# fgvieira/ngsLD

Measured on AMD Instinct MI355X. Metric: SNP-pair EM-LD computations/sec @ n_ind=500, higher is better.
Workload: dtype f64

## Files before the change

include/ngsld.h:

```cpp
#ifndef NGSLD_H
#define NGSLD_H

#include <stddef.h>
#include <stdint.h>

#ifdef __cplusplus
extern "C" {
#endif

typedef struct ngsld_ctx ngsld_ctx;

enum {
  NGSLD_OK = 0,
  NGSLD_ERR_INVALID = -1,
  NGSLD_ERR_DEVICE = -2,
  NGSLD_ERR_NOMEM = -3,
  NGSLD_ERR_NAN = -4,
  NGSLD_ERR_MAF_RANGE = -5,
  NGSLD_ERR_SINK = -6,
  NGSLD_ERR_UNSUPPORTED = -7
};

typedef struct {
  uint64_t max_kb_dist;
// ... 19 lines not shown
  uint32_t n_iter;
} ngsld_rec_ext;

typedef struct {
  uint32_t s1, s2_begin, count, reserved;
  uint64_t mask;
  uint64_t first_record;
} ngsld_item;

typedef struct {
  uint64_t s1_begin, s1_end;
  uint64_t n_pairs;
  uint64_t n_items;
  const ngsld_item *items;
  const ngsld_rec_std *std;
  const ngsld_rec_ext *ext;
  const char *text;
  uint64_t text_len;
} ngsld_batch;

typedef int (*ngsld_sink_fn)(void *user, const ngsld_batch *batch);

typedef int (*ngsld_read_sites_fn)(void *user, uint64_t site_begin, uint64_t n_sites, double *dst);

const char *ngsld_version(void);

int ngsld_create(int device, ngsld_ctx **ctx);
void ngsld_destroy(ngsld_ctx *ctx);
const char *ngsld_last_error(const ngsld_ctx *ctx);

int ngsld_set_geno_raw(ngsld_ctx *ctx, const double *gl_raw, uint64_t n_sites, uint64_t n_ind, int log_scale,
                       int ignore_miss_data, int on_device);
typedef struct {
  int32_t log_scale;
  int32_t ignore_miss_data;
  int32_t on_device;
  int32_t text_semantics;
  int32_t call_geno;
  int32_t per_individual_only;
  double N_thresh;
  double call_thresh;
} ngsld_geno_opts;
int ngsld_set_geno_raw_opts(ngsld_ctx *ctx, const double *gl_raw, uint64_t n_sites, uint64_t n_ind,
                            const ngsld_geno_opts *opts);
int ngsld_set_geno_lkl(ngsld_ctx *ctx, const double *geno_lkl, const double *maf, uint64_t n_sites, uint64_t n_ind,
                       int on_device);
int ngsld_get_maf(ngsld_ctx *ctx, double *maf_out);
int ngsld_set_pos_dist(ngsld_ctx *ctx, const double *pos_dist);

int ngsld_plan(ngsld_ctx *ctx, const ngsld_params *params, uint64_t *n_pairs);
int ngsld_plan_rows(ngsld_ctx *ctx, const uint64_t **row_off, const uint32_t **row_end);

int ngsld_run(ngsld_ctx *ctx, uint64_t s1_begin, uint64_t s1_end, ngsld_sink_fn sink, void *user);

int ngsld_set_text_output(ngsld_ctx *ctx, const char *const *labels, int enable);

int ngsld_reserve_text_buffers(ngsld_ctx *ctx, uint64_t bytes_per_row);

int ngsld_set_replay_source(ngsld_ctx *ctx, ngsld_read_sites_fn read, void *user);
int ngsld_set_replay_matrix(ngsld_ctx *ctx, const double *values);
int ngsld_set_replay(ngsld_ctx *ctx, int enable);
int ngsld_replay_stats(ngsld_ctx *ctx, uint64_t *pairs, uint64_t *sites);

int ngsld_set_exact_store(ngsld_ctx *ctx, int mode);
typedef struct {
  uint64_t pairs_flagged;
  uint64_t pairs_replayed;
  uint64_t pairs_on_device;
  uint64_t pairs_on_host;
  uint64_t sites_reevaluated;
  int32_t exact_store;
  int32_t text_rows_patched;
  double exact_store_build_s;
  uint64_t sites_degenerate;
} ngsld_replay_stats_t;
int ngsld_replay_info(ngsld_ctx *ctx, ngsld_replay_stats_t *out);

int ngsld_run_device(ngsld_ctx *ctx, uint64_t s1_begin, uint64_t s1_end, void *d_std, void *d_ext, void *hip_stream);
int ngsld_finish_device(ngsld_ctx *ctx);

int ngsld_last_kernel_time(ngsld_ctx *ctx, double *total_ms, uint64_t *n_launches, uint64_t *n_pairs);

const char *ngsld_pair_kernel(const ngsld_ctx *ctx);
int ngsld_describe_dispatch(uint64_t n_ind, int ignore_miss_data, char *buf, size_t buf_len);

int ngsld_set_tuning(ngsld_ctx *ctx, uint32_t pairs_per_item, uint64_t batch_pairs);

int ngsld_selftest(ngsld_ctx *ctx);

int ngsld_selftest_format(ngsld_ctx *ctx, uint64_t n, const ngsld_rec_std *std, const ngsld_rec_ext *ext, const double *dist,
                          const double *maf1, const double *maf2, char *text, uint64_t text_cap, uint64_t *row_len,
                          int32_t *needs_host);
int ngsld_selftest_printed(ngsld_ctx *ctx, uint64_t n, const double *x, int32_t precision, int32_t weight_type,
                           double min_weight, int64_t *micro, int32_t *micro_ok, int64_t *label, int32_t *label_rc);

typedef struct {
  uint64_t row_begin, row_end;
  uint64_t site_end;
} ngsld_slab;

int ngsld_window_ends(const double *pos_dist, uint64_t n_sites, const ngsld_params *params, uint32_t *row_end);

int ngsld_plan_slabs(const double *pos_dist, uint64_t n_sites, const ngsld_params *params, uint64_t max_slab_sites,
                     ngsld_slab *slabs, uint64_t cap, uint64_t *n_slabs);

uint64_t ngsld_slab_sites_for_budget(uint64_t n_ind, uint64_t budget_bytes);
uint64_t ngsld_sites_for_budget(uint64_t n_ind, uint64_t budget_bytes, int matrix_copies);

int ngsld_streamed_replay_info(ngsld_replay_stats_t *out);

int ngsld_set_memory_budget(int device, uint64_t bytes);

int ngsld_device_memory(int device, uint64_t *free_bytes, uint64_t *total_bytes);


int ngsld_run_streamed(int device, uint64_t n_sites, uint64_t n_ind, const double *pos_dist,
                       const ngsld_params *params, const ngsld_geno_opts *opts, uint64_t max_slab_sites,
                       ngsld_read_sites_fn read, void *read_user, double *maf_out, ngsld_sink_fn sink,
                       void *sink_user, uint64_t *n_pairs, uint64_t *n_slabs, char *err, size_t errlen);

int ngsld_run_streamed_text(int device, uint64_t n_sites, uint64_t n_ind, const double *pos_dist,
                            const ngsld_params *params, const ngsld_geno_opts *opts, uint64_t max_slab_sites,
                            ngsld_read_sites_fn read, void *read_user, double *maf_out, ngsld_sink_fn sink,
                            void *sink_user, uint64_t *n_pairs, uint64_t *n_slabs, char *err, size_t errlen,
                            const char *const *labels, int text_output);


int ngsld_plan_parts(const double *pos_dist, uint64_t n_sites, const ngsld_params *params, int n_parts, ngsld_slab *parts);

typedef int (*ngsld_multi_sink_fn)(void *user, int part, const ngsld_batch *batch);

int ngsld_run_multi(const int *devices, int n_devices, uint64_t n_sites, uint64_t n_ind, const double *pos_dist,
                    const ngsld_params *params, const ngsld_geno_opts *opts, const double *gl_raw,
                    ngsld_read_sites_fn read, void *read_user, double *maf_out, ngsld_multi_sink_fn sink, void *sink_user,
                    const char *const *labels, int text_output, uint64_t *pairs_per_part, char *err, size_t errlen);

enum { NGSLD_DIST_NONE = 0, NGSLD_DIST_UPLOAD = 1, NGSLD_DIST_PEER_COPY = 2, NGSLD_DIST_RCCL = 3 };
int ngsld_multi_last_distribution(void);

int ngsld_rccl_selftest(int device, uint64_t bytes, char *err, size_t errlen);

typedef struct {
  uint32_t struct_size;
  int32_t field;
  double max_kb_dist;
  double min_weight;
  int32_t weight_type;
  int32_t keep_heavy;
  int32_t precision;
  int32_t reserved;
  const char *const *subset;
  uint64_t n_subset;
} ngsld_prune_params;

typedef struct {
  uint32_t struct_size;
  uint32_t reserved;
  uint64_t pairs;
  uint64_t nodes, edges;
  uint64_t kept, excluded;
  uint64_t rounds;
  uint64_t host_nodes, host_edges, host_steps;
  double pairs_ms, edges_ms, graph_ms, rounds_ms, host_ms, total_ms;
} ngsld_prune_stats;

int ngsld_prune(ngsld_ctx *ctx, const ngsld_prune_params *params, const char *const *labels, uint8_t *site_state,
// ... 105 lines not shown
```

ngsld_amd/capi.py:

```python
from __future__ import annotations

import ctypes as C
import os
import subprocess

import numpy as np

PKG_DIR = os.path.dirname(os.path.abspath(__file__))
REPO_DIR = os.path.dirname(PKG_DIR)
LIB_PATH = os.environ.get("NGSLD_LIB") or os.path.join(PKG_DIR, "libngsld.so")
CLI_PATH = os.path.join(PKG_DIR, "bin", "ngsLD")

OK, ERR_INVALID, ERR_DEVICE, ERR_NOMEM, ERR_NAN, ERR_MAF_RANGE, ERR_SINK, ERR_UNSUPPORTED = 0, -1, -2, -3, -4, -5, -6, -7


class Params(C.Structure):
    _fields_ = [("max_kb_dist", C.c_uint64), ("max_snp_dist", C.c_uint64), ("min_maf", C.c_double),
                ("ignore_miss_data", C.c_int32), ("extend_out", C.c_int32), ("rnd_sample", C.c_double),
                ("seed", C.c_uint64), ("first_row", C.c_uint64)]


class GenoOpts(C.Structure):
    _fields_ = [("log_scale", C.c_int32), ("ignore_miss_data", C.c_int32), ("on_device", C.c_int32),
                ("text_semantics", C.c_int32), ("call_geno", C.c_int32), ("per_individual_only", C.c_int32),
                ("N_thresh", C.c_double), ("call_thresh", C.c_double)]


REC_STD = np.dtype([("r2_ExpG", "<f8"), ("D", "<f8"), ("Dp", "<f8"), ("r2", "<f8")])
REC_EXT = np.dtype([("hap", "<f8", (4,)), ("n_ind_data", "<u4"), ("n_iter", "<u4")])


ITEM = np.dtype([("s1", "<u4"), ("s2_begin", "<u4"), ("count", "<u4"), ("reserved", "<u4"), ("mask", "<u8"),
                 ("first_record", "<u8")])


class Batch(C.Structure):
    _fields_ = [("s1_begin", C.c_uint64), ("s1_end", C.c_uint64), ("n_pairs", C.c_uint64), ("n_items", C.c_uint64),
                ("items", C.c_void_p), ("std", C.c_void_p), ("ext", C.c_void_p), ("text", C.c_void_p),
                ("text_len", C.c_uint64)]


def items_to_pairs(items: np.ndarray) -> tuple[np.ndarray, np.ndarray]:
    if len(items) == 0:
        return np.zeros(0, dtype=np.uint64), np.zeros(0, dtype=np.uint64)
    bits = (items["mask"][:, None] >> np.arange(64, dtype=np.uint64)[None, :]) & np.uint64(1)
    bits &= (np.arange(64)[None, :] < items["count"][:, None]).astype(np.uint64)
    idx, c = np.nonzero(bits)
    return items["s1"][idx].astype(np.uint64), (items["s2_begin"][idx].astype(np.uint64) + c.astype(np.uint64))


def items_from_pairs(s1: np.ndarray, s2: np.ndarray, span: int = 64) -> np.ndarray:
    s1, s2 = np.asarray(s1, dtype=np.int64), np.asarray(s2, dtype=np.int64)
    chunk = (s2 - s1 - 1) // span
    key = s1 * (1 << 32) + chunk
    uniq, first, inv = np.unique(key, return_index=True, return_inverse=True)
    items = np.zeros(len(uniq), dtype=ITEM)
    items["s1"] = s1[first]
    items["s2_begin"] = s1[first] + 1 + chunk[first] * span
    items["first_record"] = first
    np.bitwise_or.at(items["mask"], inv, np.uint64(1) << (s2 - items["s2_begin"][inv]).astype(np.uint64))
    last = np.zeros(len(uniq), dtype=np.int64)
    np.maximum.at(last, inv, s2 - items["s2_begin"][inv].astype(np.int64))
    items["count"] = last + 1
    return items


SINK_FN = C.CFUNCTYPE(C.c_int, C.c_void_p, C.POINTER(Batch))
MULTI_SINK_FN = C.CFUNCTYPE(C.c_int, C.c_void_p, C.c_int, C.POINTER(Batch))
READ_FN = C.CFUNCTYPE(C.c_int, C.c_void_p, C.c_uint64, C.c_uint64, C.c_void_p)
SLAB = np.dtype([("row_begin", "<u8"), ("row_end", "<u8"), ("site_end", "<u8")])

SYMBOLS = [
    "ngsld_version", "ngsld_create", "ngsld_destroy", "ngsld_last_error", "ngsld_set_geno_raw",
    "ngsld_set_geno_raw_opts", "ngsld_set_geno_lkl",
    "ngsld_get_maf", "ngsld_set_pos_dist", "ngsld_plan", "ngsld_plan_rows", "ngsld_run", "ngsld_run_device", "ngsld_set_text_output",
    "ngsld_set_replay_source", "ngsld_set_replay_matrix", "ngsld_set_replay", "ngsld_replay_stats", "ngsld_finish_device",
    "ngsld_set_exact_store", "ngsld_replay_info",
    "ngsld_plan_parts", "ngsld_run_multi", "ngsld_multi_last_distribution", "ngsld_rccl_selftest",
    "ngsld_last_kernel_time", "ngsld_pair_kernel", "ngsld_describe_dispatch", "ngsld_set_tuning", "ngsld_selftest", "ngsld_selftest_format",
    "ngsld_selftest_printed", "ngsld_reserve_text_buffers",
    "ngsld_window_ends", "ngsld_plan_slabs", "ngsld_slab_sites_for_budget", "ngsld_sites_for_budget", "ngsld_streamed_replay_info", "ngsld_set_memory_budget", "ngsld_device_memory", "ngsld_run_streamed", "ngsld_run_streamed_text",
    "ngsld_host_read_geno_bin_range",
    "ngsld_host_set_threads", "ngsld_host_read_pos", "ngsld_host_pos_dist", "ngsld_host_label", "ngsld_host_free_pos", "ngsld_host_pos_slice",
    "ngsld_host_geno_size_ok", "ngsld_host_read_geno_bin", "ngsld_host_read_geno_text", "ngsld_host_format_header", "ngsld_host_format_pair",
    "ngsld_host_format_double", "ngsld_host_write_batch", "ngsld_host_replay_pair", "ngsld_host_missing_call_log",
    "ngsld_host_gz_open", "ngsld_host_gz_close",
    "ngsld_prune", "ngsld_host_prune_graph", "ngsld_host_prune_label",
    "ngsld_decay", "ngsld_decay_bins", "ngsld_host_decay_fit",
    "ngsld_blocks", "ngsld_blocks_sites", "ngsld_blocks_matrix", "ngsld_blocks_text",
    "ngsld_site_ld", "ngsld_site_ld_get",
    "ngsld_clusters", "ngsld_clusters_sites", "ngsld_clusters_table",
]


class ReplayStats(C.Structure):
    _fields_ = [("pairs_flagged", C.c_uint64), ("pairs_replayed", C.c_uint64), ("pairs_on_device", C.c_uint64),
                ("pairs_on_host", C.c_uint64), ("sites_reevaluated", C.c_uint64), ("exact_store", C.c_int32),
                ("text_rows_patched", C.c_int32), ("exact_store_build_s", C.c_double), ("sites_degenerate", C.c_uint64)]


class PruneParams(C.Structure):
    _fields_ = [("struct_size", C.c_uint32), ("field", C.c_int32), ("max_kb_dist", C.c_double), ("min_weight", C.c_double),
                ("weight_type", C.c_int32), ("keep_heavy", C.c_int32), ("precision", C.c_int32), ("reserved", C.c_int32),
                ("subset", C.POINTER(C.c_char_p)), ("n_subset", C.c_uint64)]


class PruneStats(C.Structure):
    _fields_ = [("struct_size", C.c_uint32), ("reserved", C.c_uint32), ("pairs", C.c_uint64), ("nodes", C.c_uint64),
                ("edges", C.c_uint64), ("kept", C.c_uint64), ("excluded", C.c_uint64), ("rounds", C.c_uint64),
                ("host_nodes", C.c_uint64), ("host_edges", C.c_uint64), ("host_steps", C.c_uint64),
                ("pairs_ms", C.c_double), ("edges_ms", C.c_double), ("graph_ms", C.c_double), ("rounds_ms", C.c_double),
                ("host_ms", C.c_double), ("total_ms", C.c_double)]


class DecayParams(C.Structure):
    _fields_ = [("struct_size", C.c_uint32), ("fields", C.c_uint32), ("bin_size", C.c_double), ("max_kb_dist", C.c_double),
                ("min_maf", C.c_double)]


class DecayStats(C.Structure):
    _fields_ = [("struct_size", C.c_uint32), ("lds", C.c_uint32), ("pairs", C.c_uint64), ("pairs_counted", C.c_uint64),
                ("bins", C.c_uint64), ("bin_slots", C.c_uint64), ("chunks", C.c_uint64), ("pairs_ms", C.c_double),
                ("bin_ms", C.c_double), ("total_ms", C.c_double)]


class BlocksParams(C.Structure):
    _fields_ = [("struct_size", C.c_uint32), ("fields", C.c_uint32), ("chr", C.c_char_p), ("start", C.c_uint64),
                ("end", C.c_uint64)]


class BlocksStats(C.Structure):
    _fields_ = [("struct_size", C.c_uint32), ("reserved", C.c_uint32), ("members", C.c_uint64), ("sites", C.c_uint64),
                ("pairs", C.c_uint64), ("pairs_in_region", C.c_uint64), ("cells_na", C.c_uint64), ("host_rows", C.c_uint64),
                ("chunks", C.c_uint64), ("pairs_ms", C.c_double), ("scatter_ms", C.c_double), ("format_ms", C.c_double),
                ("total_ms", C.c_double)]


class SiteLdParams(C.Structure):
    _fields_ = [("struct_size", C.c_uint32), ("fields", C.c_uint32), ("max_kb_dist", C.c_double), ("min_maf", C.c_double),
                ("linked_min", C.c_double), ("abs_value", C.c_int32), ("reserved", C.c_int32)]


class SiteLdStats(C.Structure):
    _fields_ = [("struct_size", C.c_uint32), ("lds", C.c_uint32), ("pairs", C.c_uint64), ("pairs_counted", C.c_uint64),
                ("sites_with_pairs", C.c_uint64), ("chunks", C.c_uint64), ("pairs_ms", C.c_double), ("site_ms", C.c_double),
                ("total_ms", C.c_double)]


class ClustersParams(C.Structure):
    _fields_ = [("struct_size", C.c_uint32), ("field", C.c_int32), ("max_kb_dist", C.c_double), ("min_maf", C.c_double),
                ("min_weight", C.c_double), ("abs_value", C.c_int32), ("reserved", C.c_int32)]


class ClustersStats(C.Structure):
    _fields_ = [("struct_size", C.c_uint32), ("reserved", C.c_uint32), ("pairs", C.c_uint64), ("nodes", C.c_uint64),
                ("edges", C.c_uint64), ("clusters", C.c_uint64), ("clusters_multi", C.c_uint64), ("largest", C.c_uint64),
                ("chunks", C.c_uint64), ("union_launches", C.c_uint64), ("pairs_ms", C.c_double), ("union_ms", C.c_double),
                ("finish_ms", C.c_double), ("total_ms", C.c_double)]


TEXT_FN = C.CFUNCTYPE(C.c_int, C.c_void_p, C.c_void_p, C.c_uint64)


class DecayFitResult(C.Structure):
    _fields_ = [("rate", C.c_double), ("ld_max", C.c_double), ("ld_min", C.c_double), ("sse", C.c_double),
                ("n_bins", C.c_uint64)]


DECAY_FIELDS = ("r2_ExpG", "D", "Dp", "r2")


class NgsldError(RuntimeError):
    def __init__(self, code: int, msg: str):
        super().__init__(f"ngsld error {code}: {msg}")
        self.code = code
        self.msg = msg


def build(force: bool = False, jobs: int = 8) -> None:
    csrc = os.path.join(PKG_DIR, "csrc")
    if force:
        subprocess.check_call(["make", "-s", "-C", csrc, "clean"])
    subprocess.check_call(["make", "-s", f"-j{jobs}", "-C", csrc, "all"])


_lib = None


def lib() -> C.CDLL:
    global _lib
    if _lib is None:
        if not os.path.exists(LIB_PATH):
            raise FileNotFoundError(f"{LIB_PATH} is missing: run ngsld_amd.capi.build() (or make -C ngsld_amd/csrc); "
                                    "there is no fallback implementation")
        L = C.CDLL(LIB_PATH)
        vp, u64, dbl = C.c_void_p, C.c_uint64, C.c_double
        L.ngsld_version.restype = C.c_char_p
        L.ngsld_create.argtypes = [C.c_int, C.POINTER(vp)]
        L.ngsld_destroy.argtypes = [vp]
        L.ngsld_destroy.restype = None
        L.ngsld_last_error.argtypes = [vp]
        L.ngsld_last_error.restype = C.c_char_p
        L.ngsld_set_geno_raw.argtypes = [vp, vp, u64, u64, C.c_int, C.c_int, C.c_int]
        L.ngsld_set_geno_raw_opts.argtypes = [vp, vp, u64, u64, C.POINTER(GenoOpts)]
        L.ngsld_set_geno_lkl.argtypes = [vp, vp, vp, u64, u64, C.c_int]
        L.ngsld_get_maf.argtypes = [vp, vp]
        L.ngsld_set_pos_dist.argtypes = [vp, vp]
        L.ngsld_plan.argtypes = [vp, C.POINTER(Params), C.POINTER(u64)]
        L.ngsld_plan_rows.argtypes = [vp, C.POINTER(C.POINTER(C.c_uint64)), C.POINTER(C.POINTER(C.c_uint32))]
        L.ngsld_run.argtypes = [vp, u64, u64, SINK_FN, vp]
        L.ngsld_run_device.argtypes = [vp, u64, u64, vp, vp, vp]
        if hasattr(L, "ngsld_set_replay_source"):
            L.ngsld_set_replay_source.argtypes = [vp, READ_FN, vp]
            if hasattr(L, "ngsld_set_replay_matrix"):
                L.ngsld_set_replay_matrix.argtypes = [vp, vp]
            L.ngsld_set_replay.argtypes = [vp, C.c_int]
            L.ngsld_replay_stats.argtypes = [vp, C.POINTER(u64), C.POINTER(u64)]
        if hasattr(L, "ngsld_replay_info"):
            L.ngsld_set_exact_store.argtypes = [vp, C.c_int]
            L.ngsld_replay_info.argtypes = [vp, C.POINTER(ReplayStats)]
            L.ngsld_finish_device.argtypes = [vp]
        if hasattr(L, "ngsld_set_text_output"):
            L.ngsld_set_text_output.argtypes = [vp, C.POINTER(C.c_char_p), C.c_int]
        L.ngsld_last_kernel_time.argtypes = [vp, C.POINTER(dbl), C.POINTER(u64), C.POINTER(u64)]
        L.ngsld_set_tuning.argtypes = [vp, C.c_uint32, u64]
        if hasattr(L, "ngsld_pair_kernel"):
            L.ngsld_pair_kernel.argtypes = [vp]
            L.ngsld_pair_kernel.restype = C.c_char_p
        L.ngsld_selftest.argtypes = [vp]
        if hasattr(L, "ngsld_selftest_format"):
            L.ngsld_selftest_format.argtypes = [vp, u64, vp, vp, vp, vp, vp, C.c_char_p, u64, vp, C.POINTER(C.c_int32)]
            L.ngsld_selftest_printed.argtypes = [vp, u64, vp, C.c_int32, C.c_int32, dbl, vp, vp, vp, vp]
        L.ngsld_window_ends.argtypes = [vp, u64, C.POINTER(Params), vp]
        L.ngsld_plan_slabs.argtypes = [vp, u64, C.POINTER(Params), u64, vp, u64, C.POINTER(u64)]
        L.ngsld_slab_sites_for_budget.argtypes = [u64, u64]
        L.ngsld_slab_sites_for_budget.restype = u64
        if hasattr(L, "ngsld_sites_for_budget"):
            L.ngsld_sites_for_budget.argtypes = [u64, u64, C.c_int]
            L.ngsld_sites_for_budget.restype = u64
        L.ngsld_device_memory.argtypes = [C.c_int, C.POINTER(u64), C.POINTER(u64)]
        L.ngsld_run_streamed.argtypes = [C.c_int, u64, u64, vp, C.POINTER(Params), C.POINTER(GenoOpts), u64, READ_FN, vp,
                                         vp, SINK_FN, vp, C.POINTER(u64), C.POINTER(u64), C.c_char_p, C.c_size_t]
        if hasattr(L, "ngsld_run_multi"):
            L.ngsld_plan_parts.argtypes = [vp, u64, C.POINTER(Params), C.c_int, vp]
            L.ngsld_run_multi.argtypes = [C.POINTER(C.c_int), C.c_int, u64, u64, vp, C.POINTER(Params), C.POINTER(GenoOpts),
                                          vp, READ_FN, vp, vp, MULTI_SINK_FN, vp, C.POINTER(C.c_char_p), C.c_int,
                                          C.POINTER(u64), C.c_char_p, C.c_size_t]
        if hasattr(L, "ngsld_multi_last_distribution"):
            L.ngsld_multi_last_distribution.argtypes = []
        if hasattr(L, "ngsld_rccl_selftest"):
            L.ngsld_rccl_selftest.argtypes = [C.c_int, u64, C.c_char_p, C.c_size_t]
        L.ngsld_host_read_geno_bin_range.argtypes = [C.c_char_p, u64, u64, u64, vp, C.c_char_p, C.c_size_t]
        L.ngsld_host_set_threads.argtypes = [C.c_int]
        L.ngsld_host_set_threads.restype = None
        L.ngsld_host_read_pos.argtypes = [C.c_char_p, C.c_int, u64, C.POINTER(vp), C.c_char_p, C.c_size_t]
        L.ngsld_host_pos_dist.argtypes = [vp]
        L.ngsld_host_pos_dist.restype = C.POINTER(dbl)
        L.ngsld_host_label.argtypes = [vp, u64]
        L.ngsld_host_label.restype = C.c_char_p
        L.ngsld_host_free_pos.argtypes = [vp]
        L.ngsld_host_free_pos.restype = None
        L.ngsld_host_pos_slice.argtypes = [vp, u64, u64]
        L.ngsld_host_pos_slice.restype = vp
        L.ngsld_host_geno_size_ok.argtypes = [u64, u64, u64]
        L.ngsld_host_read_geno_bin.argtypes = [C.c_char_p, u64, u64, vp, C.c_char_p, C.c_size_t]
        L.ngsld_host_read_geno_text.argtypes = [C.c_char_p, C.c_int, C.c_int, u64, u64, vp, C.POINTER(C.c_int),
                                                C.c_char_p, C.c_size_t]
        L.ngsld_host_format_header.argtypes = [C.c_char_p, C.c_size_t, C.c_int]
        L.ngsld_host_format_header.restype = C.c_size_t
        L.ngsld_host_format_pair.argtypes = [C.c_char_p, C.c_size_t, C.c_char_p, C.c_char_p, dbl, vp, vp, dbl, dbl]
        L.ngsld_host_format_pair.restype = C.c_size_t
        L.ngsld_host_format_double.argtypes = [C.c_char_p, C.c_size_t, dbl, C.c_int]
        L.ngsld_host_format_double.restype = C.c_size_t
        L.ngsld_host_write_batch.argtypes = [C.POINTER(Batch), vp, vp, vp, C.c_int, C.c_int]
        L.ngsld_host_replay_pair.argtypes = [vp, vp, u64, C.POINTER(GenoOpts), vp, vp, vp]
        if hasattr(L, "ngsld_host_gz_open"):
            L.ngsld_host_gz_open.argtypes = [C.c_char_p, C.c_int, C.POINTER(vp), C.POINTER(C.c_int)]
            L.ngsld_host_gz_close.argtypes = [vp]
        if hasattr(L, "ngsld_prune"):
            L.ngsld_prune.argtypes = [vp, C.POINTER(PruneParams), C.POINTER(C.c_char_p), vp, C.POINTER(PruneStats)]
            L.ngsld_host_prune_graph.argtypes = [u64, vp, u64, vp, vp, vp, C.c_int, vp, C.POINTER(u64)]
            L.ngsld_host_prune_label.argtypes = [dbl, C.c_int, C.c_char, C.POINTER(C.c_int64)]
        if hasattr(L, "ngsld_decay"):
            L.ngsld_decay.argtypes = [vp, C.POINTER(DecayParams), C.POINTER(DecayStats)]
            L.ngsld_decay_bins.argtypes = [vp, u64, vp, vp, vp, C.POINTER(u64)]
            L.ngsld_host_decay_fit.argtypes = [u64, vp, vp, C.c_int, dbl, dbl, C.POINTER(DecayFitResult)]
        if hasattr(L, "ngsld_blocks"):
            L.ngsld_blocks.argtypes = [vp, C.POINTER(BlocksParams), C.POINTER(C.c_char_p), C.POINTER(BlocksStats)]
            L.ngsld_blocks_sites.argtypes = [vp, u64, vp, C.POINTER(u64)]
            L.ngsld_blocks_matrix.argtypes = [vp, C.c_int, vp, vp]
            L.ngsld_blocks_text.argtypes = [vp, C.c_int, TEXT_FN, vp, C.POINTER(BlocksStats)]
        if hasattr(L, "ngsld_site_ld"):
            L.ngsld_site_ld.argtypes = [vp, C.POINTER(SiteLdParams), C.POINTER(SiteLdStats)]
            L.ngsld_site_ld_get.argtypes = [vp, C.c_int, vp, vp, vp, vp, vp]
        if hasattr(L, "ngsld_clusters"):
            L.ngsld_clusters.argtypes = [vp, C.POINTER(ClustersParams), C.POINTER(ClustersStats)]
            L.ngsld_clusters_sites.argtypes = [vp, vp]
            L.ngsld_clusters_table.argtypes = [vp, u64, u64, vp, vp, vp, vp, vp, vp, vp, vp, vp, C.POINTER(u64)]
        _lib = L
    return _lib


def prune_label(x: float, prec: int = 4, weight_type: str = "a") -> int | None:
    out = C.c_int64()
    rc = lib().ngsld_host_prune_label(float(x), prec, weight_type.encode(), C.byref(out))
    if rc == ERR_INVALID:
        return None
    if rc != OK:
        raise NgsldError(rc, "label out of range")
    return out.value


def decay_fit(dist, values, field: str = "r2", n_ind: float = 0, recomb_rate: float = 1.0) -> dict:
    d = np.ascontiguousarray(dist, dtype=np.float64)
    v = np.ascontiguousarray(values, dtype=np.float64)
    if d.shape != v.shape or d.ndim != 1:
        raise ValueError("dist and values must be 1-D arrays of one length")
# ... 541 lines not shown
                    exts.append(np.frombuffer(C.string_at(b.ext, n * REC_EXT.itemsize), dtype=REC_EXT).copy())
            items = np.frombuffer(C.string_at(b.items, b.n_items * ITEM.itemsize), dtype=ITEM) if b.n_items else \
                np.zeros(0, dtype=ITEM)
            a, bb = items_to_pairs(items)
            assert len(a) == n
            if len(items):
                assert np.array_equal(items["first_record"], np.concatenate([[0], np.cumsum(
                    [bin(int(m)).count("1") for m in items["mask"]])[:-1]]).astype(np.uint64))
            s1s.append(a)
            s2s.append(bb)
            return 0

        cb = SINK_FN(sink)
        self._check(self._L.ngsld_run(self._h, s1_begin, s1_end, cb, None))
        cat = lambda xs, dt: np.concatenate(xs) if xs else np.zeros(0, dtype=dt)
        return (cat(s1s, np.uint64), cat(s2s, np.uint64), cat(stds, REC_STD),
                cat(exts, REC_EXT) if self.extend_out else None)

    def run_to_fd(self, s1_begin: int, s1_end: int, fd: int, pos_handle, pos_dist: np.ndarray | None, maf: np.ndarray,
                  n_threads: int) -> int:
        maf = np.ascontiguousarray(maf, dtype=np.float64)
        pd_ptr = None if pos_dist is None else np.ascontiguousarray(pos_dist, dtype=np.float64).ctypes.data
        total, rc_box = [0], [0]

        libc = C.CDLL(None, use_errno=True)
        libc.write.argtypes = [C.c_int, C.c_void_p, C.c_size_t]
        libc.write.restype = C.c_ssize_t

        def sink(_user, bp):
            b = bp.contents
            total[0] += b.n_pairs
            if b.text:
                off = 0
                while off < b.text_len:
                    w = libc.write(fd, b.text + off, min(b.text_len - off, 1 << 30))
                    if w <= 0:
                        return 1
                    off += w
                return 0
            rc_box[0] = self._L.ngsld_host_write_batch(bp, pos_handle, pd_ptr, maf.ctypes.data, n_threads, fd)
            return 0 if rc_box[0] == OK else 1

        self._check(self._L.ngsld_run(self._h, s1_begin, s1_end, SINK_FN(sink), None))
        return total[0]

    def set_text_output(self, labels: list[str] | None, enable: bool = True) -> None:
        arr = None
        if labels is not None:
            arr = (C.c_char_p * len(labels))(*[l.encode() for l in labels])
        self._check(self._L.ngsld_set_text_output(self._h, arr, int(enable)))

    def run_text(self, s1_begin: int = 0, s1_end: int | None = None) -> tuple[bytes, int]:
        s1_end = self.n_sites if s1_end is None else s1_end
        parts, fallbacks = [], [0]

        def sink(_user, bp):
            b = bp.contents
            if b.text:
                parts.append(C.string_at(b.text, b.text_len))
            else:
                fallbacks[0] += 1
            return 0

        self._check(self._L.ngsld_run(self._h, s1_begin, s1_end, SINK_FN(sink), None))
        return b"".join(parts), fallbacks[0]

    def run_discard(self, s1_begin: int = 0, s1_end: int | None = None) -> int:
        s1_end = self.n_sites if s1_end is None else s1_end
        total = [0]

        def sink(_user, bp):
            total[0] += bp.contents.n_pairs
            return 0

        self._check(self._L.ngsld_run(self._h, s1_begin, s1_end, SINK_FN(sink), None))
        return total[0]

    def run_device(self, s1_begin: int, s1_end: int, d_std: int, d_ext: int | None, stream: int | None = None) -> None:
        self._check(self._L.ngsld_run_device(self._h, s1_begin, s1_end, d_std, d_ext, stream))

    def pair_kernel(self) -> str:
        return self._L.ngsld_pair_kernel(self._h).decode()

    def last_kernel_time(self) -> tuple[float, int, int]:
        ms, nl, npairs = C.c_double(), C.c_uint64(), C.c_uint64()
        self._check(self._L.ngsld_last_kernel_time(self._h, C.byref(ms), C.byref(nl), C.byref(npairs)))
        return ms.value, nl.value, npairs.value

    def prune(self, labels: list[str] | None, field: int = 7, max_kb_dist: float = float("inf"), min_weight: float = 0.0,
              weight_type: str = "a", keep_heavy: bool = False, subset: list[str] | None = None,
              precision: int = 4) -> tuple[np.ndarray, dict]:
        arr = None if labels is None else (C.c_char_p * len(labels))(*[l.encode() for l in labels])
        sub = None if subset is None else (C.c_char_p * max(len(subset), 1))(*[l.encode() for l in subset])
        p = PruneParams(C.sizeof(PruneParams), field, float(max_kb_dist), float(min_weight), ord(weight_type), int(keep_heavy),
                        precision, 0, sub, 0 if subset is None else len(subset))
        st = PruneStats()
        st.struct_size = C.sizeof(PruneStats)
        state = np.zeros(max(self.n_sites, 1), dtype=np.uint8)
        self._check(self._L.ngsld_prune(self._h, C.byref(p), arr, state.ctypes.data, C.byref(st)))
        return state[:self.n_sites], {k: getattr(st, k) for k, _ in PruneStats._fields_ if k not in ("struct_size", "reserved")}

    def decay(self, ld=("r2",), bin_size: float = 250, max_kb_dist: float = float("inf"),
              min_maf: float = 0.0) -> tuple[dict, dict]:
        ld = (ld,) if isinstance(ld, str) else tuple(ld)
        bad = [f for f in ld if f not in DECAY_FIELDS]
        if bad or not ld:
            raise ValueError(f"ld must name some of {DECAY_FIELDS}: {bad}")
        mask = sum(1 << DECAY_FIELDS.index(f) for f in set(ld))
        names = [f for k, f in enumerate(DECAY_FIELDS) if (mask >> k) & 1]
        p = DecayParams(C.sizeof(DecayParams), mask, float(bin_size), float(max_kb_dist), float(min_maf))
        st = DecayStats()
        st.struct_size = C.sizeof(DecayStats)
        self._check(self._L.ngsld_decay(self._h, C.byref(p), C.byref(st)))
        nb = st.bins
        dist = np.zeros(max(nb, 1))
        cnt = np.zeros(max(nb, 1), dtype=np.uint64)
        mean = np.zeros((max(nb, 1), len(names)))
        got = C.c_uint64()
        self._check(self._L.ngsld_decay_bins(self._h, nb, dist.ctypes.data, cnt.ctypes.data, mean.ctypes.data, C.byref(got)))
        assert got.value == nb
        bins = {"dist": dist[:nb], "n": cnt[:nb]}
        for k, f in enumerate(names):
            bins[f] = mean[:nb, k].copy()
        return bins, {k: getattr(st, k) for k, _ in DecayStats._fields_ if k != "struct_size"}

    def site_ld(self, ld=("r2",), max_kb_dist: float = float("inf"), min_maf: float = 0.0, linked_min: float = 0.5,
                abs_value: bool = True) -> tuple[dict, dict]:
        ld = (ld,) if isinstance(ld, str) else tuple(ld)
        bad = [f for f in ld if f not in DECAY_FIELDS]
        if bad or not ld:
            raise ValueError(f"ld must name some of {DECAY_FIELDS}: {bad}")
        mask = sum(1 << DECAY_FIELDS.index(f) for f in set(ld))
        p = SiteLdParams(C.sizeof(SiteLdParams), mask, float(max_kb_dist), float(min_maf), float(linked_min), int(bool(abs_value)), 0)
        st = SiteLdStats()
        st.struct_size = C.sizeof(SiteLdStats)
        self._check(self._L.ngsld_site_ld(self._h, C.byref(p), C.byref(st)))
        m = max(self.n_sites, 1)
        sites = {"n": np.zeros(m, dtype=np.uint64)}
        for k, f in enumerate(DECAY_FIELDS):
            if not (mask >> k) & 1:
                continue
            sites[f"sum_{f}"], sites[f"max_{f}"] = np.zeros(m, dtype=np.int64), np.zeros(m, dtype=np.int64)
            sites[f"linked_{f}"], sites[f"mean_{f}"] = np.zeros(m, dtype=np.uint64), np.zeros(m)
            self._check(self._L.ngsld_site_ld_get(self._h, 4 + k, sites["n"].ctypes.data, sites[f"sum_{f}"].ctypes.data,
                                                  sites[f"max_{f}"].ctypes.data, sites[f"linked_{f}"].ctypes.data,
                                                  sites[f"mean_{f}"].ctypes.data))
        sites = {k: v[:self.n_sites] for k, v in sites.items()}
        return sites, {k: getattr(st, k) for k, _ in SiteLdStats._fields_ if k != "struct_size"}

    def clusters(self, field: int = 7, min_weight: float = 0.5, max_kb_dist: float = float("inf"), min_maf: float = 0.0,
                 abs_value: bool = True, min_size: int = 2) -> tuple[np.ndarray, dict, dict]:
        p = ClustersParams(C.sizeof(ClustersParams), int(field), float(max_kb_dist), float(min_maf), float(min_weight),
                           int(bool(abs_value)), 0)
        st = ClustersStats()
        st.struct_size = C.sizeof(ClustersStats)
        self._check(self._L.ngsld_clusters(self._h, C.byref(p), C.byref(st)))
        ids = np.zeros(max(self.n_sites, 1), dtype=np.uint32)
        self._check(self._L.ngsld_clusters_sites(self._h, ids.ctypes.data))
        rows = C.c_uint64(0)
        self._check(self._L.ngsld_clusters_table(self._h, int(min_size), 0, None, None, None, None, None, None, None, None, None,
                                                 C.byref(rows)))
        m = max(int(rows.value), 1)
        kinds = dict(id=np.uint32, size=np.uint32, first=np.uint32, last=np.uint32, span=np.uint64, edges=np.uint64, sum=np.int64,
                     mean=np.float64, density=np.float64)
        table = {k: np.zeros(m, dtype=t) for k, t in kinds.items()}
        self._check(self._L.ngsld_clusters_table(self._h, int(min_size), m, *(table[k].ctypes.data for k in kinds), C.byref(rows)))
# ... 46 lines not shown
```

ngsld_amd/csrc/engine.h:

```cpp
#pragma once

#include "knobs.h"

#include <hip/hip_runtime.h>
#include <sched.h>
#include <dlfcn.h>
#include <sys/mman.h>

#include <algorithm>
#include <atomic>
#include <chrono>
#include <cmath>
#include <condition_variable>
#include <functional>
#include <cstdio>
#include <cstdlib>
#include <cstring>
#include <limits>
#include <mutex>
#include <new>
#include <string>
#include <thread>
#include <unordered_map>
#include <vector>

#include "../../include/ngsld.h"
#include "ld_common.h"
#include "ld_dispatch.h"
#include "ld_mean.h"
#include "ld_prep.h"
#include "ld_replay.h"
#include "ld_text.h"
#include "replay.h"
#include "taus.h"

namespace ngsld {
namespace eng {
extern thread_local std::string g_create_error;

struct Roctx {
  int (*push)(const char *) = nullptr;
  int (*pop)() = nullptr;
  Roctx() {
    if (const char *e = std::getenv("NGSLD_ROCTX"))
      if (std::strcmp(e, "0") == 0) return;
    for (const char *name : {"librocprofiler-sdk-roctx.so.1", "librocprofiler-sdk-roctx.so", "libroctx64.so.4", "libroctx64.so"}) {
      void *lib = dlopen(name, RTLD_NOW | RTLD_GLOBAL | RTLD_NOLOAD);
      if (lib == nullptr && std::getenv("NGSLD_ROCTX") != nullptr) lib = dlopen(name, RTLD_NOW | RTLD_GLOBAL);
      if (lib == nullptr) continue;
      push = reinterpret_cast<int (*)(const char *)>(dlsym(lib, "roctxRangePushA"));
      pop = reinterpret_cast<int (*)()>(dlsym(lib, "roctxRangePop"));
      if (push && pop) return;
      push = nullptr;
      pop = nullptr;
    }
  }
};
inline Roctx &roctx() {
  static Roctx r;
  return r;
}
struct Range {
  bool on;
  explicit Range(const char *name) : on(roctx().push != nullptr) {
    if (on) roctx().push(name);
  }
  ~Range() {
    if (on) roctx().pop();
  }
  Range(const Range &) = delete;
  Range &operator=(const Range &) = delete;
};

template <typename T>
struct DevBuf {
  T *p = nullptr;
  size_t n = 0;
  DevBuf() = default;
  DevBuf(const DevBuf &) = delete;
  DevBuf &operator=(const DevBuf &) = delete;
  ~DevBuf() { release(); }
  hipError_t resize(size_t count) {
    if (count <= n && p != nullptr) return hipSuccess;
    release();
    if (count == 0) return hipSuccess;
    hipError_t e = hipMalloc((void **)&p, count * sizeof(T));
    if (e == hipSuccess) n = count;
    return e;
  }
  void release() {
    if (p) (void)hipFree(p);
    p = nullptr;
    n = 0;
  }
};

template <typename T>
struct PinBuf {
  T *p = nullptr;
  size_t n = 0;
  void *map_base = nullptr;
  size_t map_len = 0;
  PinBuf() = default;
  PinBuf(const PinBuf &) = delete;
  PinBuf &operator=(const PinBuf &) = delete;
  ~PinBuf() { release(); }
  hipError_t resize(size_t count) {
    if (count <= n && p != nullptr) return hipSuccess;
    release();
    if (count == 0) return hipSuccess;
    const size_t huge = (size_t)2 << 20, want = count * sizeof(T);
// ... 54 lines not shown
    while ((int)threads_.size() < T - 1) {
      const int id = (int)threads_.size() + 1;
      threads_.emplace_back([this, id] { loop(id); });
    }
    {
      std::lock_guard<std::mutex> lk(mu_);
      job_ = [&fn](int t) { fn(t); };
      n_ = T;
      left_ = T - 1;
      ++epoch_;
    }
    cv_.notify_all();
    fn(0);
    std::unique_lock<std::mutex> lk(mu_);
    done_.wait(lk, [this] { return left_ == 0; });
    job_ = nullptr;
  }

 private:
  void loop(int id) {
    uint64_t seen = 0;
    for (;;) {
      std::function<void(int)> job;
      {
        std::unique_lock<std::mutex> lk(mu_);
        cv_.wait(lk, [&] { return stop_ || epoch_ != seen; });
        if (stop_) return;
        seen = epoch_;
        if (id >= n_) continue;
        job = job_;
      }
      job(id);
      std::lock_guard<std::mutex> lk(mu_);
      if (--left_ == 0) done_.notify_all();
    }
  }
  std::vector<std::thread> threads_;
  std::mutex mu_;
  std::condition_variable cv_, done_;
  std::function<void(int)> job_;
  int n_ = 0, left_ = 0;
  uint64_t epoch_ = 0;
  bool stop_ = false;
};

}
}

using namespace ngsld;
using namespace ngsld::eng;

struct FlagRow {
  uint64_t rec, off;
  uint32_t len, s1, s2, pad;
};
constexpr uint32_t kFlagRowsCap = 1024;

struct ngsld_ctx {
  int device = 0;
  hipStream_t stream = nullptr, stream2 = nullptr, copy_stream = nullptr;
  hipStream_t text_stream = nullptr;
  hipEvent_t ev_scan_done[3] = {nullptr, nullptr, nullptr};
  std::string err;

  uint64_t n_sites = 0, n_ind = 0;
  uint32_t np = 0;
  PairConfig cfg{};
  bool have_geno = false;
  DevBuf<double> d_planes, d_maf, d_mean, d_rsx, d_sc4;
  DevBuf<int> d_status;
  std::vector<double> h_maf, h_pos_dist;
  DevBuf<uint64_t> d_hard_masks;
  DevBuf<double> d_hard_u;
  DevBuf<int> d_all_hard, d_odd_missing;
  int h_odd_missing = 0;
  bool missing_canonical = false;
  int h_all_hard = 0, h_prep_status = 0;
  uint32_t mask_words = 0;
  DevBuf<uint8_t> d_skip;
  DevBuf<uint32_t> d_skip_count;
  uint32_t h_skip_count = 0;
  bool skip_on = true;
  bool skip_kernels = false;

  bool planned = false;
  ngsld_params params{};
  std::vector<uint64_t> h_row_off, h_item_off;
  std::vector<uint32_t> h_row_end;
  std::vector<uint8_t> h_keep;
  std::vector<Item> h_items;
  std::vector<uint64_t> h_run_off;
  uint64_t run_len = 0;
  std::vector<uint64_t> run_ends;
  int n_cus = 256;
  DevBuf<Run> d_runs;
  DevBuf<uint64_t> d_row_off, d_item_off, d_row_seed, d_row_count;
  DevBuf<uint32_t> d_row_end;
  DevBuf<uint8_t> d_keep;
  DevBuf<Item> d_items;
  uint64_t n_items = 0;

  int kernel_choice = kChooseAuto;
  uint32_t pairs_per_item = 16;
  uint64_t batch_pairs = 1ull << 23;
  bool batch_pairs_set = false;

  static constexpr int kSlots = 3;
  DevBuf<ngsld_rec_std> d_std[kSlots];
  DevBuf<ngsld_rec_ext> d_ext[kSlots];
  PinBuf<ngsld_rec_std> h_std[kSlots];
  PinBuf<ngsld_rec_ext> h_ext[kSlots];
  hipEvent_t ev_kernel_done[kSlots] = {nullptr, nullptr, nullptr}, ev_copy_done[kSlots] = {nullptr, nullptr, nullptr};
  bool run_direct = true, run_taper = true;
  int run_streams = 1;
  bool timed_overlap = false;

  bool text_mode = false, have_labels = false;
  uint64_t max_label = 6;
  DevBuf<char> d_labels, d_text[kSlots], d_scan_tmp, d_scan_tmp_b;
  DevBuf<uint64_t> d_label_off, d_lens[kSlots], d_offs[kSlots], d_text_meta[kSlots];
  DevBuf<double> d_cum;
  DevBuf<uint32_t> d_infc;
  PinBuf<char> h_text[kSlots];
  PinBuf<uint64_t> h_text_meta[kSlots];
  std::thread reserve_thread;

  bool replay_on = true;
  ngsld_read_sites_fn replay_read = nullptr;
  void *replay_user = nullptr;
  const double *replay_matrix = nullptr;
  std::mutex replay_mu;
  hipStream_t replay_stream = nullptr;
  std::mutex replay_stream_mu;
  ngsld_geno_opts gopts{};
  bool normalised = false;
  DevBuf<uint32_t> d_flags[kSlots], d_flags_dev;
  PinBuf<uint32_t> h_flags[kSlots], h_flags_dev;
  PinBuf<uint32_t> h_flag_bits;
  PinBuf<FlagRow> h_flag_rows[kSlots];
  uint32_t flag_cap[kSlots] = {0, 0, 0}, flag_cap_dev = 0;
  bool replay_device = true;
  uint64_t replayed_on_device = 0;
  uint64_t text_rows_patched = 0;
  DevBuf<double> d_xplanes, d_xmaf;
  DevBuf<double> d_xT;
  std::atomic<bool> xT_ready{false};
  DevBuf<uint32_t> d_xperm;
  DevBuf<uint32_t> d_xdepth;
  struct LaneScratch {
    DevBuf<ReplayEntry> list;
    DevBuf<uint64_t> keys_a, keys_b;
    DevBuf<uint32_t> vals_a, vals_b;
    DevBuf<char> temp;
    void release() { list.release(); keys_a.release(); keys_b.release(); vals_a.release(); vals_b.release(); temp.release(); }
  } lane_scratch[kSlots], lane_scratch_dev;
  PinBuf<double> h_xstage[2];
  std::thread exact_thread;
  std::atomic<int> exact_state{0};
  std::atomic<uint64_t> exact_frontier{0};
  std::atomic<bool> exact_cancel{false};
  std::mutex exact_mu;
  std::condition_variable exact_cv;
  int exact_rc = 0;
  std::string exact_msg;
  hipStream_t exact_stream = nullptr;
  ReplayPool exact_pool;
// ... 56 lines not shown
    bool valid = false;
    std::vector<uint32_t> id, size, first, last;
    std::vector<uint64_t> span, edges;
    std::vector<int64_t> sum;
    std::vector<double> mean, density;
  } clusters;
  void clear_clusters() { clusters = Clusters(); }

  uint32_t blocks_fields = 0;
  uint64_t blocks_members = 0;
  DevBuf<double> d_blocks_val;
  DevBuf<uint8_t> d_blocks_present;
  DevBuf<uint32_t> d_blocks_col;
  std::vector<uint64_t> blocks_site;
  std::vector<std::string> blocks_label;
  DevBuf<char> d_blocks_label;
  DevBuf<uint64_t> d_blocks_label_off;
  void clear_blocks() {
    clear_sites();
    clear_clusters();
    blocks_fields = 0;
    blocks_members = 0;
    d_blocks_val.release();
    d_blocks_present.release();
    d_blocks_col.release();
    d_blocks_label.release();
    d_blocks_label_off.release();
    blocks_site.clear();
    blocks_label.clear();
  }
};

namespace ngsld {
namespace eng {


inline int fail(ngsld_ctx *c, int code, const std::string &msg) {
  if (c) c->err = msg;
  return code;
}

inline int hip_fail(ngsld_ctx *c, hipError_t e, const char *what) {
  return fail(c, e == hipErrorOutOfMemory ? NGSLD_ERR_NOMEM : NGSLD_ERR_DEVICE,
              std::string(what) + ": " + hipGetErrorString(e));
}

#define HIP_TRY(c, call)                                \
  do {                                                  \
    hipError_t e_ = (call);                             \
    if (e_ != hipSuccess) return hip_fail(c, e_, #call); \
  } while (0)

inline int caught(ngsld_ctx *c, bool nomem) {
  if (c) {
    (void)hipSetDevice(c->device);
    (void)hipDeviceSynchronize();
    c->planned = false;
  }
  return nomem ? fail(c, NGSLD_ERR_NOMEM, "out of host memory") : fail(c, NGSLD_ERR_INVALID, "unexpected C++ exception");
}
#define NGSLD_CATCH(ctx)                                        \
  catch (const std::bad_alloc &) { return caught(ctx, true); }  \
  catch (...) { return caught(ctx, false); }

inline int check_status(ngsld_ctx *c) {
  int status = 0;
  HIP_TRY(c, hipMemcpy(&status, c->d_status.p, sizeof(int), hipMemcpyDeviceToHost));
  if (status == NGSLD_ERR_MAF_RANGE) return fail(c, NGSLD_ERR_MAF_RANGE, "invalid allele frequencies");
  return NGSLD_OK;
}

constexpr uint64_t kTextBatchPairs = 1ull << 19;

inline uint32_t flag_cap_for(uint64_t n) { return (uint32_t)std::min<uint64_t>(1ull << 20, std::max<uint64_t>(4096, n / 256)); }
inline size_t flag_head_bytes(uint32_t cap) { return (size_t)flag_head_words(cap) * sizeof(uint32_t); }
inline size_t flag_bitmap_words(uint64_t n) { return (size_t)((n + 31) / 32); }
inline size_t flag_words(uint64_t n, uint32_t cap) { return (size_t)flag_head_words(cap) + 2 * flag_bitmap_words(n); }

void plan_rows(const std::vector<double> &pos_dist, const std::vector<double> &maf, const ngsld_params &p, uint64_t n,
               std::vector<uint32_t> &row_end);
int build_runs(ngsld_ctx *c, uint64_t run_len, const std::vector<uint64_t> &launch_ends);

hipError_t timed_launch(ngsld_ctx *c, const PairArgs &a, hipStream_t stream);
PairArgs make_args(ngsld_ctx *c, uint64_t r0, uint64_t r1, ngsld_rec_std *d_std, ngsld_rec_ext *d_ext,
                   uint32_t *d_flags = nullptr, uint32_t flag_cap = 0, uint64_t flag_n = 0);

bool dist_prefix(const ngsld_ctx *c, std::vector<double> &cum, std::vector<uint32_t> &infc);

constexpr uint64_t kRecordChunkPairs = 1ull << 24;
inline uint64_t record_chunk(const char *knob) {
  return knob ? std::max<uint64_t>(1, std::min<uint64_t>(kRecordChunkPairs, std::strtoull(knob, nullptr, 10))) : kRecordChunkPairs;
}
uint64_t record_cap(const ngsld_ctx *c, uint64_t chunk, const uint8_t *rows = nullptr);

int run_record_chunks(ngsld_ctx *c, uint64_t chunk_pairs, ngsld_rec_std *d_rec, uint64_t rec_cap, double *pairs_ms,
                      const std::function<int(uint64_t r0, uint64_t r1, uint64_t pairs)> &on_chunk, const uint8_t *rows = nullptr);

struct EventPair {
  hipEvent_t a = nullptr, b = nullptr;
  EventPair() = default;
  EventPair(const EventPair &) = delete;
  EventPair &operator=(const EventPair &) = delete;
  ~EventPair() {
    if (a) (void)hipEventDestroy(a);
    if (b) (void)hipEventDestroy(b);
  }
  hipError_t create() {
    hipError_t e = hipEventCreate(&a);
    return e == hipSuccess ? hipEventCreate(&b) : e;
  }
  hipError_t add_elapsed(double *ms) const {
    float t = 0.f;
    const hipError_t e = hipEventElapsedTime(&t, a, b);
    if (e == hipSuccess) *ms += t;
    return e;
  }
};

int launch_record_items(ngsld_ctx *c, EventPair &ev, uint64_t r0, uint64_t r1, double *ms, uint64_t *chunks,
                        const std::function<void(const ngsld_item *items, uint64_t n_items)> &launch);

inline unsigned blocks_for(uint64_t threads, unsigned per_block = 256) { return (unsigned)((threads + per_block - 1) / per_block); }
inline double ms_since(std::chrono::steady_clock::time_point t0) {
  return std::chrono::duration<double, std::milli>(std::chrono::steady_clock::now() - t0).count();
}
template <class P, class S>
int check_struct_sizes(ngsld_ctx *c, const P *p, const char *p_name, const S *stats, const char *s_name) {
  if (p == nullptr || p->struct_size != sizeof(P))
    return fail(c, NGSLD_ERR_INVALID, std::string(p_name) + ": struct_size must be sizeof(" + p_name + ")");
  if (stats != nullptr && stats->struct_size < sizeof(uint32_t)) return fail(c, NGSLD_ERR_INVALID, std::string(s_name) + ": struct_size not set");
  return NGSLD_OK;
}
template <class S>
void copy_stats(S *out, const S &s) {
  if (out == nullptr) return;
  const uint32_t want = out->struct_size;
  std::memcpy(out, &s, std::min<size_t>(want, sizeof(S)));
  out->struct_size = want;
}
inline int field_list(uint32_t mask, int field[4]) {
  int ns = 0;
  for (int f = 0; f < 4; ++f)
    if ((mask >> f) & 1u) field[ns++] = f;
  return ns;
}

int send_flag_rows(ngsld_ctx *c, const uint32_t *d_flags, uint32_t cap, bool dev_applied, const uint64_t *d_offs, const uint64_t *d_lens,
                   uint64_t n_records, uint64_t base, FlagRow *h_rows, hipStream_t st);
int replay_pairs_on_host(ngsld_ctx *c, const uint32_t *s1, const uint32_t *s2, size_t n, ngsld_rec_std *out_std, ngsld_rec_ext *out_ext);
unsigned usable_threads();
hipStream_t replay_stream_of(ngsld_ctx *c);
int ensure_host_items(ngsld_ctx *c);
int fetch_replay_site(ngsld_ctx *c, uint64_t s, std::vector<double> &tmp, ReplaySite *out);
int flagged_records(ngsld_ctx *c, const uint32_t *h_head, const uint32_t *d_flags, uint32_t cap, uint64_t n,
                    std::vector<uint64_t> &recs, bool dev_applied = false);
bool room_for(uint64_t need_bytes, uint64_t device_margin, uint64_t budget_margin);
bool lkl_device_eligible(const ngsld_ctx *c);
bool exact_store_is_free(const ngsld_ctx *c);
inline bool exact_store_started(const ngsld_ctx *c) { return c->exact_state.load() >= 1; }
int start_exact_store(ngsld_ctx *c);
int reserve_device_run(ngsld_ctx *c, uint64_t n_records);
int wait_exact_store(ngsld_ctx *c, uint64_t need_sites, bool *have);
int ensure_exact_store(ngsld_ctx *c);
void stop_exact_store(ngsld_ctx *c);
inline uint64_t exact_sites_needed(const ngsld_ctx *c, uint64_t r0, uint64_t r1) {
  uint64_t need = r1;
// ... 20 lines not shown
```

ngsld_amd/csrc/engine.hip:

```cpp
#include "engine.h"

#include <atomic>

namespace ngsld {
namespace eng {

thread_local std::string g_create_error;

int set_geno_common(ngsld_ctx *c, const double *gl, const double *maf, uint64_t n_sites, uint64_t n_ind,
                    const ngsld_geno_opts &o, bool normalised) {
  if (c == nullptr) return NGSLD_ERR_INVALID;
  const int log_scale = o.log_scale, ignore_miss = o.ignore_miss_data, on_device = o.on_device;
  Range range_("ngsld:set_geno (upload + per-site prep)");
  if (o.call_geno && o.N_thresh > o.call_thresh)
    return fail(c, NGSLD_ERR_INVALID, "missing data threshold must be smaller than calling genotype threshold!");
  if (gl == nullptr || n_sites == 0 || n_ind == 0) return fail(c, NGSLD_ERR_INVALID, "empty genotype matrix");
  if (normalised && maf == nullptr) return fail(c, NGSLD_ERR_INVALID, "maf missing");
  if (n_sites >= 0xffffffffull) return fail(c, NGSLD_ERR_UNSUPPORTED, "n_sites must be below 2^32 - 1");
  PairConfig cfg;
  if (!pair_config(n_ind, &cfg, c->kernel_choice, ignore_miss != 0))
    return fail(c, NGSLD_ERR_UNSUPPORTED, "n_ind is outside the supported range");
  HIP_TRY(c, hipSetDevice(c->device));
  (void)hipGetLastError();
  {
    const int rcp = finish_device_run(c);
    if (rcp != NGSLD_OK) return rcp;
  }
  stop_exact_store(c);
  c->have_geno = false;
  c->planned = false;
  c->clear_blocks();
  c->text_mode = false;
  c->replay_read = nullptr;
  c->replay_user = nullptr;
  c->replay_matrix = nullptr;
  c->exact_ready = false;
  c->exact_alias = false;
  c->exact_failed = false;
  c->exact_build_s = 0.0;
  c->host_replayed_total = 0;
  c->d_xplanes.release();
  c->d_xmaf.release();
  c->d_xT.release();
  c->d_xdepth.release();
  c->d_xperm.release();
  c->xT_ready = false;
  for (int k = 0; k < 2; ++k) {
    c->d_group_std[k].release();
    c->d_group_ext[k].release();
  }
  c->d_group_lens.release();
  c->d_group_offs.release();
  c->d_group_text.release();
  c->gopts = o;
  c->normalised = normalised;
  c->n_sites = n_sites;
  c->n_ind = n_ind;
  c->cfg = cfg;
  c->np = cfg.np;
  const bool trace = std::getenv("NGSLD_TRACE") != nullptr;
  const auto t_0 = std::chrono::steady_clock::now();
  auto ms_since = [&]() { return std::chrono::duration<double, std::milli>(std::chrono::steady_clock::now() - t_0).count(); };
  const size_t plane_elems = (size_t)n_sites * 3 * c->np;
  HIP_TRY(c, c->d_planes.resize(plane_elems));
  HIP_TRY(c, c->d_maf.resize(n_sites));
  HIP_TRY(c, c->d_mean.resize(n_sites));
  HIP_TRY(c, c->d_rsx.resize(n_sites));
  HIP_TRY(c, c->d_sc4.resize(4 * n_sites));
  HIP_TRY(c, c->d_status.resize(1));
  HIP_TRY(c, hipMemsetAsync(c->d_status.p, 0, sizeof(int), c->stream));

  PrepArgs a{};
  a.planes = c->d_planes.p;
  a.site_stride = 3ull * c->np;
  a.np = c->np;
  a.n_ind = (uint32_t)n_ind;
  a.log_scale = log_scale;
  a.ignore_miss = ignore_miss;
  a.normalised_input = normalised ? 1 : 0;
  a.text_semantics = o.text_semantics;
  a.call_geno = o.call_geno;
  {
    const char *pe = test_knob("PREP_EXACT");
    a.exact_chain = (pe != nullptr && std::strcmp(pe, "0") != 0) ? 1 : 0;
  }
  a.N_thresh = o.N_thresh;
  a.call_thresh = o.call_thresh;
  a.maf = c->d_maf.p;
  a.mean_e = c->d_mean.p;
  a.rsx = c->d_rsx.p;
  a.status = c->d_status.p;
  c->missing_canonical = false;
  const bool look_for_odd_missing = o.text_semantics && log_scale && !o.call_geno && !normalised;
  if (look_for_odd_missing) {
    HIP_TRY(c, c->d_odd_missing.resize(1));
    HIP_TRY(c, hipMemsetAsync(c->d_odd_missing.p, 0, sizeof(int), c->stream));
    a.odd_missing = c->d_odd_missing.p;
    a.missing_canon = replay_missing_raw_text();
  }
  if (on_device) {
    a.raw = gl;
    a.maf_in = maf;
    a.site0 = 0;
    a.n_sites = n_sites;
    HIP_TRY(c, launch_prep(a, c->stream));
  } else {
    const uint64_t site_bytes = n_ind * 3 * sizeof(double);
    uint64_t stage_bytes = 64ull << 20;
    if (const char *e = test_knob("STAGE_BYTES")) stage_bytes = std::strtoull(e, nullptr, 10);
    uint64_t chunk = stage_bytes / site_bytes;
    if (chunk < 1) chunk = 1;
    if (chunk > n_sites) chunk = n_sites;
    DevBuf<double> stage[2], maf_stage[2];
    hipEvent_t prepped[2] = {nullptr, nullptr};
    for (int k = 0; k < 2; ++k) {
      HIP_TRY(c, stage[k].resize(chunk * n_ind * 3));
      if (normalised) HIP_TRY(c, maf_stage[k].resize(chunk));
      HIP_TRY(c, hipEventCreateWithFlags(&prepped[k], hipEventDisableTiming));
    }
    int rc = NGSLD_OK;
    uint64_t k = 0;
    if (trace) std::fprintf(stderr, "[trace] set_geno: device buffers + staging allocated at %.2f ms\n", ms_since());
    for (uint64_t s0 = 0; s0 < n_sites && rc == NGSLD_OK; s0 += chunk, ++k) {
      const int b = (int)(k & 1);
      const uint64_t m = std::min(chunk, n_sites - s0);
      hipError_t e = hipSuccess;
      if (k >= 2) e = hipEventSynchronize(prepped[b]);
      if (e == hipSuccess)
        e = hipMemcpyAsync(stage[b].p, gl + s0 * n_ind * 3, m * site_bytes, hipMemcpyHostToDevice, c->copy_stream);
      if (e == hipSuccess && normalised)
        e = hipMemcpyAsync(maf_stage[b].p, maf + s0, m * sizeof(double), hipMemcpyHostToDevice, c->copy_stream);
      if (e == hipSuccess) e = hipStreamSynchronize(c->copy_stream);
      if (trace) std::fprintf(stderr, "[trace] set_geno: chunk %llu (%llu sites) on the device at %.2f ms\n", (unsigned long long)k, (unsigned long long)m, ms_since());
      a.raw = stage[b].p;
      a.maf_in = normalised ? maf_stage[b].p : nullptr;
      a.site0 = s0;
      a.n_sites = m;
      if (e == hipSuccess) e = launch_prep(a, c->stream);
      if (e == hipSuccess) e = hipEventRecord(prepped[b], c->stream);
      if (e != hipSuccess) rc = hip_fail(c, e, "chunked genotype upload");
    }
    hipError_t e = hipStreamSynchronize(c->stream);
    if (trace) std::fprintf(stderr, "[trace] set_geno: last prep kernel done at %.2f ms\n", ms_since());
    for (int q = 0; q < 2; ++q) {
      stage[q].release();
      maf_stage[q].release();
      if (prepped[q]) (void)hipEventDestroy(prepped[q]);
    }
    if (trace) std::fprintf(stderr, "[trace] set_geno: staging buffers freed at %.2f ms\n", ms_since());
    if (rc != NGSLD_OK) return rc;
    if (e != hipSuccess) return hip_fail(c, e, "chunked genotype upload");
  }
  c->h_skip_count = 0;
  const bool look_for_skip = c->skip_on && c->replay_on && c->replay_device && c->exact_mode != 0;
  c->skip_kernels = cfg.kernel == kRun || (cfg.kernel == kMulti && cfg.form == 0 && cfg.waves == 2);
  if (look_for_skip) {
    HIP_TRY(c, c->d_skip.resize(n_sites));
    HIP_TRY(c, c->d_skip_count.resize(1));
    HIP_TRY(c, hipMemsetAsync(c->d_skip_count.p, 0, sizeof(uint32_t), c->stream));
    HIP_TRY(c, launch_site_skip(c->d_planes.p, 3ull * c->np, c->np, (uint32_t)n_ind, ignore_miss, c->d_maf.p, n_sites, c->d_skip.p,
                                c->d_skip_count.p, c->stream));
    HIP_TRY(c, hipMemcpyAsync(&c->h_skip_count, c->d_skip_count.p, sizeof(uint32_t), hipMemcpyDeviceToHost, c->stream));
  } else {
    c->d_skip.release();
  }
  HIP_TRY(c, launch_pack_scalars(c->d_maf.p, c->d_mean.p, c->d_rsx.p, c->d_skip.p, c->d_sc4.p, n_sites, c->stream));
  int &all_hard = c->h_all_hard;
  all_hard = 0;
  const char *hk = test_knob("HARD_KERNEL");
  const bool try_hard = n_ind <= kHardMaxInd && !o.per_individual_only && !(hk != nullptr && std::strcmp(hk, "0") == 0);
  if (try_hard) {
    c->mask_words = (uint32_t)((n_ind + 63) / 64);
    HIP_TRY(c, c->d_hard_masks.resize((size_t)n_sites * 4 * c->mask_words));
    HIP_TRY(c, c->d_hard_u.resize(n_sites));
    HIP_TRY(c, c->d_all_hard.resize(1));
    all_hard = 1;
    HIP_TRY(c, hipMemcpyAsync(c->d_all_hard.p, &all_hard, sizeof(int), hipMemcpyHostToDevice, c->stream));
    HIP_TRY(c, launch_classify_hard(c->d_planes.p, 3ull * c->np, c->np, (uint32_t)n_ind, n_sites, c->d_hard_masks.p,
                                    c->d_hard_u.p, c->d_all_hard.p, c->stream));
    HIP_TRY(c, hipMemcpyAsync(&all_hard, c->d_all_hard.p, sizeof(int), hipMemcpyDeviceToHost, c->stream));
    if (trace) std::fprintf(stderr, "[trace] set_geno: called-genotype check enqueued at %.2f ms\n", ms_since());
  }
  c->h_maf.resize(n_sites);
  int &status = c->h_prep_status;
  status = 0;
  HIP_TRY(c, hipMemcpyAsync(c->h_maf.data(), c->d_maf.p, n_sites * sizeof(double), hipMemcpyDeviceToHost, c->stream));
  HIP_TRY(c, hipMemcpyAsync(&status, c->d_status.p, sizeof(int), hipMemcpyDeviceToHost, c->stream));
  c->h_odd_missing = 1;
  if (look_for_odd_missing)
    HIP_TRY(c, hipMemcpyAsync(&c->h_odd_missing, c->d_odd_missing.p, sizeof(int), hipMemcpyDeviceToHost, c->stream));
  HIP_TRY(c, hipStreamSynchronize(c->stream));
  c->missing_canonical = look_for_odd_missing && c->h_odd_missing == 0;
  if (trace) std::fprintf(stderr, "[trace] set_geno: scalars packed, called-genotype check, maf on the host at %.2f ms\n", ms_since());
  if (status == NGSLD_ERR_NAN) return fail(c, NGSLD_ERR_NAN, "NaN found! Is the file format correct?");
  if (try_hard && all_hard) {
    c->cfg.kernel = kHard;
    c->cfg.group = 16;
    c->cfg.slots = 1;
    c->cfg.waves = 1;
  } else {
    c->d_hard_masks.release();
    c->d_hard_u.release();
  }
  c->have_geno = true;
  return NGSLD_OK;
}
}
}

extern "C" {

const char *ngsld_version(void) { return "ngsld-amd 0.10.0 (gfx950; reference ngsLD 1.2.1)"; }

int ngsld_create(int device, ngsld_ctx **out) {
  if (out == nullptr) return NGSLD_ERR_INVALID;
  *out = nullptr;
  int n_dev = 0;
  hipError_t e = hipGetDeviceCount(&n_dev);
  if (e != hipSuccess || n_dev == 0) {
    g_create_error = std::string("no HIP device available (") + hipGetErrorString(e) +
                     "); this library has no CPU fallback";
    return NGSLD_ERR_DEVICE;
  }
  if (device < 0 || device >= n_dev) {
    g_create_error = "device index out of range";
    return NGSLD_ERR_INVALID;
  }
  hipDeviceProp_t prop;
  e = hipGetDeviceProperties(&prop, device);
  if (e != hipSuccess) {
    g_create_error = std::string("hipGetDeviceProperties: ") + hipGetErrorString(e);
    return NGSLD_ERR_DEVICE;
  }
  if (std::strncmp(prop.gcnArchName, "gfx950", 6) != 0) {
    g_create_error = std::string("device is ") + prop.gcnArchName + ", this build targets gfx950 (MI355X) only";
    return NGSLD_ERR_DEVICE;
  }
  ngsld_ctx *c = new (std::nothrow) ngsld_ctx();
  if (c == nullptr) return NGSLD_ERR_NOMEM;
  c->device = device;
  if (prop.multiProcessorCount > 0) c->n_cus = prop.multiProcessorCount;
  if (const char *k = std::getenv("NGSLD_PAIR_KERNEL")) {
    c->kernel_choice = std::strcmp(k, "multi") == 0 ? kChooseMulti
                       : (std::strcmp(k, "ab") == 0 ? kChooseAB
                          : (std::strcmp(k, "stream") == 0 ? kChoosePlainStream : (std::strcmp(k, "abm") == 0 ? kChooseABMulti
                                                               : (std::strcmp(k, "bres") == 0 ? kChooseResidentStream : kChooseAuto))));
  }
  if (const char *k = test_knob("BATCH_PAIRS")) {
    const uint64_t v = std::strtoull(k, nullptr, 10);
    if (v > 0) {
      c->batch_pairs = v;
      c->batch_pairs_set = true;
    }
  }
  if (const char *k = std::getenv("NGSLD_REPLAY")) c->replay_on = std::strcmp(k, "0") != 0;
  if (const char *k = std::getenv("NGSLD_REPLAY_THREADS")) c->replay_threads = std::atoi(k);
  if (const char *k = std::getenv("NGSLD_REPLAY_DEVICE")) c->replay_device = std::strcmp(k, "0") != 0;
  if (const char *k = std::getenv("NGSLD_REPLAY_SKIP")) c->skip_on = std::strcmp(k, "0") != 0;
  if (const char *k = std::getenv("NGSLD_EXACT_STORE")) c->exact_mode = std::max(0, std::min(2, std::atoi(k)));
  if (const char *k = test_knob("RUN_DIRECT")) c->run_direct = std::strcmp(k, "0") != 0;
  if (const char *k = test_knob("RUN_TAPER")) c->run_taper = std::strcmp(k, "0") != 0;
  if (const char *k = test_knob("RUN_STREAMS")) c->run_streams = std::atoi(k) >= 2 ? 2 : 1;
  if ((e = hipSetDevice(device)) != hipSuccess || (e = hipStreamCreate(&c->stream)) != hipSuccess ||
      (e = hipStreamCreate(&c->stream2)) != hipSuccess || (e = hipStreamCreate(&c->copy_stream)) != hipSuccess) {
    g_create_error = std::string("stream setup: ") + hipGetErrorString(e);
    delete c;
    return NGSLD_ERR_DEVICE;
  }
  for (int k = 0; k < ngsld_ctx::kSlots; ++k) {
    (void)hipEventCreateWithFlags(&c->ev_kernel_done[k], hipEventDisableTiming);
    (void)hipEventCreateWithFlags(&c->ev_copy_done[k], hipEventDisableTiming);
  }
  *out = c;
  return NGSLD_OK;
}

void ngsld_destroy(ngsld_ctx *c) {
  if (c == nullptr) return;
  if (c->reserve_thread.joinable()) c->reserve_thread.join();
  stop_exact_store(c);
  (void)hipSetDevice(c->device);
  (void)hipDeviceSynchronize();
  if (c->exact_stream) (void)hipStreamDestroy(c->exact_stream);
  c->d_planes.release(); c->d_maf.release(); c->d_mean.release(); c->d_rsx.release(); c->d_sc4.release(); c->d_runs.release(); c->d_skip.release(); c->d_skip_count.release();
  c->d_hard_masks.release(); c->d_hard_u.release(); c->d_all_hard.release();
  c->d_xplanes.release(); c->d_xmaf.release(); c->d_xT.release(); c->d_xdepth.release(); c->d_xperm.release(); c->h_xstage[0].release(); c->h_xstage[1].release();
  c->lane_scratch_dev.release();
  for (int k = 0; k < ngsld_ctx::kSlots; ++k) c->lane_scratch[k].release();
  c->d_labels.release(); c->d_scan_tmp.release(); c->d_scan_tmp_b.release(); c->d_label_off.release(); c->d_cum.release(); c->d_infc.release();
  for (int k = 0; k < ngsld_ctx::kSlots; ++k) {
    c->d_text[k].release(); c->d_lens[k].release(); c->d_offs[k].release(); c->d_text_meta[k].release();
    c->h_text[k].release(); c->h_text_meta[k].release();
  }
  c->d_status.release(); c->d_row_off.release(); c->d_item_off.release(); c->d_row_end.release();
  c->d_row_seed.release(); c->d_row_count.release(); c->d_keep.release(); c->d_items.release();
  for (int k = 0; k < ngsld_ctx::kSlots; ++k) {
    c->d_std[k].release(); c->d_ext[k].release(); c->h_std[k].release(); c->h_ext[k].release();
    if (c->ev_kernel_done[k]) (void)hipEventDestroy(c->ev_kernel_done[k]);
    if (c->ev_copy_done[k]) (void)hipEventDestroy(c->ev_copy_done[k]);
  }
  for (auto &ev : c->ev_pool) {
    (void)hipEventDestroy(ev.first);
    (void)hipEventDestroy(ev.second);
  }
  if (c->stream) (void)hipStreamDestroy(c->stream);
  if (c->stream2) (void)hipStreamDestroy(c->stream2);
  if (c->copy_stream) (void)hipStreamDestroy(c->copy_stream);
  if (c->text_stream) (void)hipStreamDestroy(c->text_stream);
  for (int k = 0; k < 3; ++k)
    if (c->ev_scan_done[k]) (void)hipEventDestroy(c->ev_scan_done[k]);
  if (c->replay_stream) (void)hipStreamDestroy(c->replay_stream);
  delete c;
}

const char *ngsld_last_error(const ngsld_ctx *c) { return c ? c->err.c_str() : g_create_error.c_str(); }

int ngsld_set_geno_raw(ngsld_ctx *c, const double *gl_raw, uint64_t n_sites, uint64_t n_ind, int log_scale,
                       int ignore_miss_data, int on_device) try {
  ngsld_geno_opts o{};
  o.log_scale = log_scale;
  o.ignore_miss_data = ignore_miss_data;
  o.on_device = on_device;
  return set_geno_common(c, gl_raw, nullptr, n_sites, n_ind, o, false);
} NGSLD_CATCH(c)

int ngsld_set_geno_raw_opts(ngsld_ctx *c, const double *gl_raw, uint64_t n_sites, uint64_t n_ind,
                            const ngsld_geno_opts *opts) try {
  if (opts == nullptr) return c ? fail(c, NGSLD_ERR_INVALID, "opts is NULL") : NGSLD_ERR_INVALID;
  return set_geno_common(c, gl_raw, nullptr, n_sites, n_ind, *opts, false);
} NGSLD_CATCH(c)

int ngsld_set_geno_lkl(ngsld_ctx *c, const double *geno_lkl, const double *maf, uint64_t n_sites, uint64_t n_ind,
                       int on_device) try {
  ngsld_geno_opts o{};
  o.on_device = on_device;
  return set_geno_common(c, geno_lkl, maf, n_sites, n_ind, o, true);
} NGSLD_CATCH(c)

int ngsld_get_maf(ngsld_ctx *c, double *maf_out) try {
  if (c == nullptr || maf_out == nullptr) return NGSLD_ERR_INVALID;
  if (!c->have_geno) return fail(c, NGSLD_ERR_INVALID, "no genotype data set");
  std::memcpy(maf_out, c->h_maf.data(), c->n_sites * sizeof(double));
  return NGSLD_OK;
} NGSLD_CATCH(c)

int ngsld_set_pos_dist(ngsld_ctx *c, const double *pos_dist) try {
  if (c == nullptr) return NGSLD_ERR_INVALID;
  if (!c->have_geno) return fail(c, NGSLD_ERR_INVALID, "set the genotype data before the positions");
  c->planned = false;
  c->clear_blocks();
  if (pos_dist == nullptr)
    c->h_pos_dist.assign(c->n_sites, std::numeric_limits<double>::infinity());
  else
    c->h_pos_dist.assign(pos_dist, pos_dist + c->n_sites);
  return NGSLD_OK;
} NGSLD_CATCH(c)
const char *ngsld_pair_kernel(const ngsld_ctx *c) {
  if (c == nullptr || !c->have_geno) return "";
  switch (effective_kernel(c->cfg, c->params.ignore_miss_data != 0)) {
    case kGroup: return "group";
    case kMulti: return c->cfg.form == 1 ? "multi-ab" : "multi";
    case kStream: return "stream";
    case kRun: return "run";
    case kHard: return "hard";
    case kRunAB: return "ab";
    default: return "";
  }
}

int ngsld_describe_dispatch(uint64_t n_ind, int ignore_miss_data, char *buf, size_t buf_len) {
  if (buf == nullptr || buf_len == 0) return NGSLD_ERR_INVALID;
  buf[0] = 0;
  PairConfig cfg;
  const bool masked = ignore_miss_data != 0;
  if (!pair_config(n_ind, &cfg, kChooseAuto, masked)) return NGSLD_ERR_UNSUPPORTED;
  const char *family = "";
  int slots = cfg.slots, waves = cfg.waves;
  switch (effective_kernel(cfg, masked)) {
    case kGroup: family = "group"; break;
    case kMulti:
      family = cfg.form == 1 ? "multi-ab" : "multi";
      if (cfg.form == 0) multi_shape(cfg, masked, &slots, &waves);
      break;
    case kStream: family = "stream"; break;
    case kRun: family = "run"; break;
    case kRunAB: family = "ab"; break;
    default: return NGSLD_ERR_UNSUPPORTED;
  }
  const int n = std::snprintf(buf, buf_len, "%s %dx%d lanes=%d np=%u", family, waves, slots, cfg.group, cfg.np);
  return (n < 0 || (size_t)n >= buf_len) ? NGSLD_ERR_INVALID : NGSLD_OK;
}

int ngsld_set_tuning(ngsld_ctx *c, uint32_t pairs_per_item, uint64_t batch_pairs) {
  if (c == nullptr) return NGSLD_ERR_INVALID;
  c->clear_blocks();
  if (pairs_per_item) {
    c->pairs_per_item = pairs_per_item;
    c->planned = false;
  }
  if (batch_pairs) {
    c->batch_pairs = batch_pairs;
    c->batch_pairs_set = true;
  }
  return NGSLD_OK;
}

int ngsld_selftest(ngsld_ctx *c) try {
  if (c == nullptr) return NGSLD_ERR_INVALID;
  HIP_TRY(c, hipSetDevice(c->device));
  (void)hipGetLastError();
  std::vector<double> in(320), out(71, 0.0);
  uint64_t st = 0x9E3779B97F4A7C15ull;
  for (auto &v : in) {
    st = st * 6364136223846793005ull + 1442695040888963407ull;
    v = (double)(st >> 11) / 9007199254740992.0 + 1e-3;
  }
  for (int l = 0; l < 64; ++l) in[256 + l] *= std::pow(10.0, -(l % 30));
  DevBuf<double> d_in, d_out;
  HIP_TRY(c, d_in.resize(in.size()));
  HIP_TRY(c, d_out.resize(out.size()));
  HIP_TRY(c, hipMemcpy(d_in.p, in.data(), in.size() * sizeof(double), hipMemcpyHostToDevice));
  HIP_TRY(c, launch_selftest(d_in.p, d_out.p, c->stream));
  HIP_TRY(c, hipStreamSynchronize(c->stream));
  HIP_TRY(c, hipMemcpy(out.data(), d_out.p, out.size() * sizeof(double), hipMemcpyDeviceToHost));
  d_in.release();
  d_out.release();
  for (int k = 0; k < 7; ++k) {
    const int v = k < 4 ? k : k - 4;
    const double got = k < 4 ? out[k] : out[68 + v];
    long double ref = 0;
    for (int l = 0; l < 64; ++l) ref += in[v * 64 + l];
    if (!(std::fabs((double)(got - ref)) <= 1e-14 * std::fabs((double)ref))) {
      char buf[160];
      std::snprintf(buf, sizeof(buf), "%s value %d: got %.17g expected %.17Lg", k < 4 ? "wave_sum4" : "wave_sum3", v, got, ref);
      return fail(c, NGSLD_ERR_DEVICE, buf);
    }
  }
  for (int l = 0; l < 64; ++l) {
    const double ref = 1.0 / in[256 + l];
    if (std::fabs(out[4 + l] - ref) > 4.5e-16 * ref) {
      char buf[160];
      std::snprintf(buf, sizeof(buf), "rcp_refined lane %d: got %.17g expected %.17g", l, out[4 + l], ref);
      return fail(c, NGSLD_ERR_DEVICE, buf);
    }
  }
  return NGSLD_OK;
} NGSLD_CATCH(c)

int ngsld_selftest_format(ngsld_ctx *c, uint64_t n, const ngsld_rec_std *std_rec, const ngsld_rec_ext *ext_rec, const double *dist,
                          const double *maf1, const double *maf2, char *text, uint64_t text_cap, uint64_t *row_len,
                          int32_t *needs_host) try {
// ... 142 lines not shown
```

ngsld_amd/csrc/engine_plan.hip:

```cpp
#include "engine.h"

namespace ngsld {
namespace eng {

void plan_rows(const std::vector<double> &pos_dist, const std::vector<double> &maf, const ngsld_params &p,
               uint64_t n, std::vector<uint32_t> &row_end) {
  row_end.assign(n, 0);
  const bool use_dist = p.max_kb_dist > 0;
  const double limit = (double)(p.max_kb_dist * 1000);
  bool exact = true;
  std::vector<double> cum;
  std::vector<uint32_t> seg;
  if (use_dist) {
    cum.assign(n, 0.0);
    seg.assign(n, 0);
    double run = 0.0;
    uint32_t sg = 0;
    for (uint64_t s = 0; s < n; ++s) {
      const double g = pos_dist[s];
      if (std::isinf(g) && g > 0) {
        if (s > 0) ++sg;
      } else if (s > 0) {
        if (!(g >= 1.0) || g != std::floor(g) || run + g > 9.0e15) exact = false;
        run += g;
// ... 30 lines not shown

int build_runs(ngsld_ctx *c, uint64_t run_len, const std::vector<uint64_t> &launch_ends) {
  run_len = std::max<uint64_t>(1, std::min<uint64_t>(run_len, kRunItems));
  if (c->run_len == run_len && c->run_ends == launch_ends) return NGSLD_OK;
  const uint64_t n = c->n_sites;
  uint64_t tail_len = std::max<uint64_t>(1, run_len / 8);
  uint64_t tail_pairs = (uint64_t)c->n_cus * run_len * item_span(c->cfg, c->pairs_per_item);
  if (const char *e = test_knob("TAIL_LEN")) tail_len = (uint64_t)std::max(0l, atol(e));
  if (const char *e = test_knob("TAIL_PAIRS")) tail_pairs = std::strtoull(e, nullptr, 10);
  std::vector<uint8_t> in_tail(n, 0);
  if (tail_len > 0 && tail_len < run_len) {
    uint64_t begin = 0;
    for (const uint64_t end : launch_ends) {
      if (end > n || end < begin) continue;
      for (uint64_t s1 = end; s1 > begin && c->h_row_off[end] - c->h_row_off[s1 - 1] <= tail_pairs; --s1) in_tail[s1 - 1] = 1;
      begin = end;
    }
  }
  std::vector<Run> runs;
  c->h_run_off.assign(n + 1, 0);
  for (uint64_t s1 = 0; s1 < n; ++s1) {
    const uint64_t i0 = c->h_item_off[s1], m = c->h_item_off[s1 + 1] - i0;
    const uint64_t len = in_tail[s1] ? tail_len : run_len;
    const uint64_t parts = (m + len - 1) / len;
    for (uint64_t q = 0; q < parts; ++q) {
      const uint64_t b = i0 + m * q / parts, e = i0 + m * (q + 1) / parts;
      runs.push_back(Run{(uint32_t)b, (uint32_t)(e - b)});
    }
    c->h_run_off[s1 + 1] = runs.size();
  }
  if (c->run_len != 0) HIP_TRY(c, hipDeviceSynchronize());
  HIP_TRY(c, c->d_runs.resize(runs.empty() ? 1 : runs.size()));
  if (!runs.empty())
    HIP_TRY(c, hipMemcpy(c->d_runs.p, runs.data(), runs.size() * sizeof(Run), hipMemcpyHostToDevice));
  c->run_len = run_len;
  c->run_ends = launch_ends;
  return NGSLD_OK;
}
}
}

extern "C" {

int ngsld_plan(ngsld_ctx *c, const ngsld_params *p, uint64_t *n_pairs) try {
  if (c == nullptr || p == nullptr) return NGSLD_ERR_INVALID;
  if (!c->have_geno) return fail(c, NGSLD_ERR_INVALID, "no genotype data set");
  if (c->h_pos_dist.size() != c->n_sites) {
    if (p->max_kb_dist > 0)
      return fail(c, NGSLD_ERR_INVALID, "position file necessary in order to filter by maximum distance!");
    c->h_pos_dist.assign(c->n_sites, std::numeric_limits<double>::infinity());
  }
  if (p->min_maf < 0 || p->min_maf > 1)
    return fail(c, NGSLD_ERR_INVALID, "minimum allele frequency must be in [0,1]!");
  HIP_TRY(c, hipSetDevice(c->device));
  (void)hipGetLastError();
  Range range_("ngsld:plan");
  {
    const int rcp = finish_device_run(c);
    if (rcp != NGSLD_OK) return rcp;
  }
  const uint64_t n = c->n_sites;
  c->params = *p;
  c->planned = false;
  c->clear_blocks();
  if (!(p->rnd_sample >= 0 && p->rnd_sample <= 1))
    return fail(c, NGSLD_ERR_INVALID, "proportion of comparisons to sample must be in ]0,1]!");
  const bool sampling = p->rnd_sample > 0 && p->rnd_sample < 1;
  c->replayed_sites = 0;
  if (c->replay_on && (c->replay_read != nullptr || c->replay_matrix != nullptr) && !c->normalised) {
    bool changed = false;
    std::vector<double> tmp;
    ReplaySite site;
    for (uint64_t s = 0; s < n; ++s) {
      const double m = c->h_maf[s], t = std::fabs(m) * 1e6;
      const bool tie = p->min_maf > 0 && std::fabs(m - p->min_maf) <= 1e-12;
      const bool edge = p->extend_out && std::fabs((t - std::floor(t)) - 0.5) < 1e-6;
      if (!tie && !edge) continue;
      const int rcs = fetch_replay_site(c, s, tmp, &site);
      if (rcs != NGSLD_OK) return fail(c, rcs, "the replay source callback failed");
      ++c->replayed_sites;
      if (site.maf != m && !(site.maf != site.maf && m != m)) {
        c->h_maf[s] = site.maf;
        changed = true;
      }
    }
    if (changed) {
      HIP_TRY(c, hipMemcpy(c->d_maf.p, c->h_maf.data(), n * sizeof(double), hipMemcpyHostToDevice));
      HIP_TRY(c, launch_pack_scalars(c->d_maf.p, c->d_mean.p, c->d_rsx.p, c->d_skip.p, c->d_sc4.p, n, c->stream));
    }
  }
  plan_rows(c->h_pos_dist, c->h_maf, *p, n, c->h_row_end);
  c->h_keep.resize(n);
  for (uint64_t s = 0; s < n; ++s) c->h_keep[s] = (c->h_maf[s] < p->min_maf) ? 0 : 1;
  const uint64_t ch = item_span(c->cfg, c->pairs_per_item);
  c->h_item_off.resize(n + 1);
  c->h_item_off[0] = 0;
  for (uint64_t s1 = 0; s1 < n; ++s1) {
    const uint64_t end = c->h_row_end[s1];
    const uint64_t span = end > s1 + 1 ? end - (s1 + 1) : 0;
    c->h_item_off[s1 + 1] = c->h_item_off[s1] + (span + ch - 1) / ch;
  }
  c->n_items = c->h_item_off[n];
  if (uses_runs(c->cfg.kernel)) {
    if (c->n_items > 0xffffffffull) return fail(c, NGSLD_ERR_UNSUPPORTED, "more than 2^32 work items in one plan");
    c->run_len = 0;
  }
  HIP_TRY(c, c->d_row_end.resize(n));
  HIP_TRY(c, c->d_keep.resize(n));
  HIP_TRY(c, c->d_row_off.resize(n + 1));
  HIP_TRY(c, c->d_item_off.resize(n + 1));
  HIP_TRY(c, c->d_row_count.resize(n));
  HIP_TRY(c, c->d_items.resize(c->n_items ? c->n_items : 1));
  HIP_TRY(c, hipMemcpyAsync(c->d_row_end.p, c->h_row_end.data(), n * sizeof(uint32_t), hipMemcpyHostToDevice, c->stream));
  HIP_TRY(c, hipMemcpyAsync(c->d_keep.p, c->h_keep.data(), n, hipMemcpyHostToDevice, c->stream));
  HIP_TRY(c, hipMemcpyAsync(c->d_item_off.p, c->h_item_off.data(), (n + 1) * sizeof(uint64_t), hipMemcpyHostToDevice, c->stream));
  std::vector<uint64_t> seeds;
  if (sampling) {
    seeds.resize(n);
    Taus master;
    master.set(p->seed);
    for (uint64_t k = 0; k < p->first_row; ++k) master.get();
    for (uint64_t s = 0; s < n; ++s) seeds[s] = master.row_seed();
    HIP_TRY(c, c->d_row_seed.resize(n));
    HIP_TRY(c, hipMemcpyAsync(c->d_row_seed.p, seeds.data(), n * sizeof(uint64_t), hipMemcpyHostToDevice, c->stream));
  }
  ItemArgs ia{};
  ia.row_end = c->d_row_end.p;
  ia.keep = c->d_keep.p;
  ia.row_seed = sampling ? c->d_row_seed.p : nullptr;
  ia.row_off = c->d_row_off.p;
  ia.item_off = c->d_item_off.p;
  ia.row_count = c->d_row_count.p;
  ia.items = c->d_items.p;
  ia.n_sites = (uint32_t)n;
  ia.span = (uint32_t)ch;
  ia.rnd_sample = p->rnd_sample;
  ia.count_only = 1;
  HIP_TRY(c, launch_items(ia, c->stream));
  std::vector<uint64_t> counts(n);
  HIP_TRY(c, hipMemcpyAsync(counts.data(), c->d_row_count.p, n * sizeof(uint64_t), hipMemcpyDeviceToHost, c->stream));
  HIP_TRY(c, hipStreamSynchronize(c->stream));
  c->h_row_off.resize(n + 1);
  c->h_row_off[0] = 0;
  for (uint64_t s1 = 0; s1 < n; ++s1) c->h_row_off[s1 + 1] = c->h_row_off[s1] + counts[s1];
  HIP_TRY(c, hipMemcpyAsync(c->d_row_off.p, c->h_row_off.data(), (n + 1) * sizeof(uint64_t), hipMemcpyHostToDevice, c->stream));
  ia.count_only = 0;
  HIP_TRY(c, launch_items(ia, c->stream));
  c->h_items.clear();
  HIP_TRY(c, hipStreamSynchronize(c->stream));
  if (uses_runs(c->cfg.kernel)) {
    const int rcr = build_runs(c, kRunItems, std::vector<uint64_t>{n});
    if (rcr != NGSLD_OK) return rcr;
  }
  c->planned = true;
  if (n_pairs) *n_pairs = c->h_row_off[n];
  return NGSLD_OK;
} NGSLD_CATCH(c)

int ngsld_plan_rows(ngsld_ctx *c, const uint64_t **row_off, const uint32_t **row_end) {
  if (c == nullptr) return NGSLD_ERR_INVALID;
  if (!c->planned) return fail(c, NGSLD_ERR_INVALID, "ngsld_plan has not been called");
  if (row_off) *row_off = c->h_row_off.data();
  if (row_end) *row_end = c->h_row_end.data();
  return NGSLD_OK;
}
int ngsld_window_ends(const double *pos_dist, uint64_t n_sites, const ngsld_params *p, uint32_t *row_end) try {
  if (p == nullptr || row_end == nullptr || n_sites == 0 || n_sites >= 0xffffffffull) return NGSLD_ERR_INVALID;
  std::vector<double> pd;
  if (pos_dist == nullptr)
    pd.assign(n_sites, std::numeric_limits<double>::infinity());
  else
// ... 12 lines not shown
```

ngsld_amd/csrc/engine_run.hip:

```cpp
#include "engine.h"
#include "../../include/ngsld_host.h"

namespace ngsld {
namespace eng {

hipError_t timed_launch(ngsld_ctx *c, const PairArgs &a, hipStream_t stream) {
  if (c->ev_used == c->ev_pool.size()) {
    hipEvent_t b, e;
    hipError_t r = hipEventCreate(&b);
    if (r != hipSuccess) return r;
    r = hipEventCreate(&e);
    if (r != hipSuccess) return r;
    c->ev_pool.emplace_back(b, e);
  }
  auto &ev = c->ev_pool[c->ev_used++];
  hipError_t r = hipEventRecord(ev.first, stream);
  if (r != hipSuccess) return r;
  r = launch_pair_kernel(c->cfg, c->params.ignore_miss_data != 0, a, stream);
  if (r != hipSuccess) return r;
  return hipEventRecord(ev.second, stream);
}

PairArgs make_args(ngsld_ctx *c, uint64_t r0, uint64_t r1, ngsld_rec_std *d_std, ngsld_rec_ext *d_ext, uint32_t *d_flags,
                   uint32_t flag_cap, uint64_t flag_n) {
  PairArgs a{};
  a.flags = d_flags;
  a.flags_host = d_flags != nullptr ? d_flags + flag_head_words(flag_cap) + flag_bitmap_words(flag_n) : nullptr;
  a.flag_cap = flag_cap;
  a.flag_text = 1;
  a.pearson_on_device = lkl_device_eligible(c) ? 1 : 0;
  a.skip_degenerate = (d_flags != nullptr && c->h_skip_count > 0 && c->skip_on && lkl_device_eligible(c) && !c->exact_failed) ? 1 : 0;
  a.planes = c->d_planes.p;
  a.site_stride = 3ull * c->np;
  a.np = c->np;
  a.n_ind = (uint32_t)c->n_ind;
  a.inv_n = 1.0 / (double)c->n_ind;
  a.maf = c->d_maf.p;
  a.mean_e = c->d_mean.p;
  a.rsx = c->d_rsx.p;
  a.items = c->d_items.p + c->h_item_off[r0];
  a.n_items = c->h_item_off[r1] - c->h_item_off[r0];
  if (uses_runs(c->cfg.kernel)) {
    a.runs = c->d_runs.p + c->h_run_off[r0];
    a.n_runs = c->h_run_off[r1] - c->h_run_off[r0];
  }
  a.hard_masks = c->d_hard_masks.p;
  a.hard_u = c->d_hard_u.p;
  a.mask_words = c->mask_words;
  a.items_all = c->d_items.p;
  a.item_off = c->d_item_off.p;
  a.h_item_off = c->h_item_off.data();
  a.row0 = (uint32_t)r0;
  a.row1 = (uint32_t)r1;
  a.planes_bytes = c->n_sites * 3ull * c->np * sizeof(double);
  a.sc4 = c->d_sc4.p;
  a.out_base = c->h_row_off[r0];
  a.out_std = d_std;
  a.out_ext = d_ext;
  a.status = c->d_status.p;
  return a;
}
}
}

extern "C" {

int ngsld_set_text_output(ngsld_ctx *c, const char *const *labels, int enable) try {
  if (c == nullptr) return NGSLD_ERR_INVALID;
  if (!c->have_geno) return fail(c, NGSLD_ERR_INVALID, "set the genotype data before the labels");
  HIP_TRY(c, hipSetDevice(c->device));
  (void)hipGetLastError();
  c->text_mode = false;
  c->clear_blocks();
  if (!enable) return NGSLD_OK;
  c->have_labels = labels != nullptr;
  c->max_label = 6;
  if (labels != nullptr) {
    std::vector<uint64_t> off(c->n_sites + 1, 0);
    for (uint64_t s = 0; s < c->n_sites; ++s) {
      if (labels[s] == nullptr) return fail(c, NGSLD_ERR_INVALID, "a label is NULL");
      const uint64_t n = std::strlen(labels[s]);
      off[s + 1] = off[s] + n;
      c->max_label = std::max<uint64_t>(c->max_label, n);
    }
    std::vector<char> blob(off[c->n_sites] ? off[c->n_sites] : 1);
    for (uint64_t s = 0; s < c->n_sites; ++s) std::memcpy(blob.data() + off[s], labels[s], off[s + 1] - off[s]);
    HIP_TRY(c, c->d_labels.resize(blob.size()));
    HIP_TRY(c, c->d_label_off.resize(c->n_sites + 1));
    HIP_TRY(c, hipMemcpy(c->d_labels.p, blob.data(), blob.size(), hipMemcpyHostToDevice));
    HIP_TRY(c, hipMemcpy(c->d_label_off.p, off.data(), off.size() * sizeof(uint64_t), hipMemcpyHostToDevice));
  }
  c->text_mode = true;
  return NGSLD_OK;
} NGSLD_CATCH(c)

int ngsld_reserve_text_buffers(ngsld_ctx *c, uint64_t bytes_per_row) try {
  if (c == nullptr) return NGSLD_ERR_INVALID;
  if (c->reserve_thread.joinable()) c->reserve_thread.join();
  if (bytes_per_row == 0) return NGSLD_OK;
  const uint64_t bytes_per_batch = bytes_per_row * std::min<uint64_t>(c->batch_pairs, kTextBatchPairs);
// ... 960 lines not shown
```

ngsld_amd/csrc/ld_common.h:

```cpp
#pragma once

#include <hip/hip_runtime.h>
#include <stdint.h>

#include "../../include/ngsld.h"

namespace ngsld {

#ifndef NGSLD_PRIO_S
#define NGSLD_PRIO_S 0
#define NGSLD_PRIO_TREE 3
#define NGSLD_PRIO_R 1
#define NGSLD_PRIO_SERIAL 3
#endif
#ifndef NGSLD_SETPRIO
#define NGSLD_SETPRIO 1
#endif
#ifndef NGSLD_MASK_SLOTS
#define NGSLD_MASK_SLOTS 6
#endif
constexpr int kIterMax = 100;
constexpr double kEpsilon = 1e-5;

constexpr double kHapNoise = 0x1p-49;
constexpr double kRecordTol = 2.5e-10;
constexpr double kReplayFloor = 0x1p-30;
constexpr double kTieMargin = 1e-12;
constexpr double kPearsonCond = 0x1p13;
constexpr double kEpsilonTie = kEpsilon + kTieMargin;
constexpr uint32_t kTieBit = 0x80000000u;
constexpr uint64_t kFlagHostOnly = 1ull << 63, kFlagDone = 1ull << 62, kFlagIndexMask = (1ull << 62) - 1;
constexpr uint32_t kFlagListAt = 8;
constexpr uint32_t kFlagHostCap = 1024;
__host__ __device__ inline uint32_t flag_head_words(uint32_t cap) { return kFlagListAt + 2u * cap + 2u * kFlagHostCap; }

typedef ngsld_item Item;

struct Run {
  uint32_t first_item, n_items;
};
#ifndef NGSLD_RUN_ITEMS
#define NGSLD_RUN_ITEMS 16
#endif
constexpr uint32_t kRunItems = NGSLD_RUN_ITEMS;

struct PairArgs {
  const double *planes;
  uint64_t site_stride;
  uint32_t np;
  uint32_t n_ind;
  double inv_n;
  const double *maf;
  const double *mean_e;
  const double *rsx;
  const Item *items;
  uint64_t n_items;
  const struct Run *runs;
  uint64_t n_runs;
  const Item *items_all;
  const double *sc4;
  uint64_t out_base;
  ngsld_rec_std *out_std;
  ngsld_rec_ext *out_ext;
  int *status;
  const uint64_t *hard_masks;
  const double *hard_u;
  uint32_t mask_words;
  uint32_t *flags;
  uint32_t *flags_host;
  uint32_t flag_cap;
  uint32_t flag_text;
  uint32_t pearson_on_device;
  uint32_t skip_degenerate;
  const uint64_t *item_off;
  const uint64_t *h_item_off;
  uint32_t row0, row1, tile_rows, tile_nk;
  uint64_t planes_bytes;
};

typedef unsigned u32x2 __attribute__((ext_vector_type(2)));

__device__ __forceinline__ double mk_double(unsigned lo, unsigned hi) { return __hiloint2double((int)hi, (int)lo); }

__device__ __forceinline__ double ref_nan(double v) { return v != v ? mk_double(0u, 0xfff80000u) : v; }

__device__ __forceinline__ double uniform(double v) {
  return mk_double((unsigned)__builtin_amdgcn_readfirstlane(__double2loint(v)),
                   (unsigned)__builtin_amdgcn_readfirstlane(__double2hiint(v)));
}

__device__ __forceinline__ double read_lane(double v, int lane) {
  return mk_double((unsigned)__builtin_amdgcn_readlane(__double2loint(v), lane),
                   (unsigned)__builtin_amdgcn_readlane(__double2hiint(v), lane));
}

__device__ __forceinline__ double fold32(double x, double y) {
  u32x2 l = __builtin_amdgcn_permlane32_swap((unsigned)__double2loint(x), (unsigned)__double2loint(y), false, false);
  u32x2 h = __builtin_amdgcn_permlane32_swap((unsigned)__double2hiint(x), (unsigned)__double2hiint(y), false, false);
  return mk_double(l[0], h[0]) + mk_double(l[1], h[1]);
}

__device__ __forceinline__ double fold16(double x, double y) {
  u32x2 l = __builtin_amdgcn_permlane16_swap((unsigned)__double2loint(x), (unsigned)__double2loint(y), false, false);
  u32x2 h = __builtin_amdgcn_permlane16_swap((unsigned)__double2hiint(x), (unsigned)__double2hiint(y), false, false);
  return mk_double(l[0], h[0]) + mk_double(l[1], h[1]);
}

template <int CTRL>
__device__ __forceinline__ double dpp_mov(double v) {
  int lo = __double2loint(v), hi = __double2hiint(v);
  lo = __builtin_amdgcn_update_dpp(0, lo, CTRL, 0xf, 0xf, true);
  hi = __builtin_amdgcn_update_dpp(0, hi, CTRL, 0xf, 0xf, true);
  return __hiloint2double(hi, lo);
}

__device__ __forceinline__ void wave_sum4(double &t0, double &t1, double &t2, double &t3) {
  double z01 = fold32(t0, t1);
  double z23 = fold32(t2, t3);
  double w = fold16(z01, z23);
  w += dpp_mov<0x128>(w);
  w += dpp_mov<0x124>(w);
  w += dpp_mov<0x4E>(w);
  w += dpp_mov<0xB1>(w);
  t0 = read_lane(w, 0);
  t2 = read_lane(w, 16);
  t1 = read_lane(w, 32);
  t3 = read_lane(w, 48);
}

template <int CTRL, int ROW_MASK>
__device__ __forceinline__ double dpp_mov_rows(double v) {
  int lo = __double2loint(v), hi = __double2hiint(v);
  lo = __builtin_amdgcn_update_dpp(0, lo, CTRL, ROW_MASK, 0xf, false);
  hi = __builtin_amdgcn_update_dpp(0, hi, CTRL, ROW_MASK, 0xf, false);
  return __hiloint2double(hi, lo);
}

__device__ __forceinline__ double wave_sum3_rows(double t1, double t2, double t3) {
  double z12 = fold32(t1, t2);
  double w = fold16(z12, t3);
  w += dpp_mov<0x128>(w);
  w += dpp_mov<0x124>(w);
  w += dpp_mov<0x4E>(w);
  w += dpp_mov<0xB1>(w);
  w += dpp_mov_rows<0x143, 0x8>(w);
  return w;
}
__device__ __forceinline__ void wave_sum3(double &t1, double &t2, double &t3) {
  double z12 = fold32(t1, t2);
  double w = fold16(z12, t3);
  w += dpp_mov<0x128>(w);
  w += dpp_mov<0x124>(w);
  w += dpp_mov<0x4E>(w);
  w += dpp_mov<0xB1>(w);
  t1 = read_lane(w, 0);
  t2 = read_lane(w, 32);
  int ulo, uhi;
  asm("; undefined" : "=v"(ulo), "=v"(uhi));
  const int lo = __builtin_amdgcn_update_dpp(ulo, __double2loint(w), 0x143, 0x8, 0xf, false);
  const int hi = __builtin_amdgcn_update_dpp(uhi, __double2hiint(w), 0x143, 0x8, 0xf, false);
// ... 87 lines not shown
```

ngsld_amd/csrc/ld_em.h:

```cpp
#pragma once

#include "ld_common.h"

namespace ngsld {

template <int N>
struct RcpTree {
  static constexpr int L = N / 2;
  static __device__ __forceinline__ double prod(const double *s) {
    return RcpTree<L>::prod(s) * RcpTree<N - L>::prod(s + L);
  }
  static __device__ __forceinline__ void down(const double *s, double inv, double *r) {
    const double pl = RcpTree<L>::prod(s), pr = RcpTree<N - L>::prod(s + L);
    RcpTree<L>::down(s, inv * pr, r);
    RcpTree<N - L>::down(s + L, inv * pl, r + L);
  }
};
template <>
struct RcpTree<1> {
  static __device__ __forceinline__ double prod(const double *s) { return s[0]; }
  static __device__ __forceinline__ void down(const double *, double inv, double *r) { r[0] = inv; }
};

struct PairedTag { static constexpr bool value = true; };
// ... 33 lines not shown
  return reinterpret_cast<const double *>((uintptr_t)(((uint64_t)hi << 32) | lo));
}

template <int SLOTS, bool MASKED, bool ONLY_LAST = false, bool UNCENTRED = false, bool A_GLOBAL = false>
__device__ __forceinline__ void stage_pair(const double *pa, uint32_t npa, uint32_t ia0, const double *pb, uint32_t npb,
                                           uint32_t ib0, uint32_t ind0, uint32_t n_ind, double mean1, double mean2,
                                           double (&P)[SLOTS][9], uint32_t &vbits, double &sxy, bool flip_a = false,
                                           bool flip_b = false, const double (*a_regs)[3] = nullptr, int n_a_regs = 0) {
  vbits = 0;
  sxy = 0.0;
  const double *pa0 = pa + (flip_a ? 2 * npa : 0u), *pa1 = pa + npa, *pa2 = pa + (flip_a ? 0u : 2 * npa);
  const double *pb0 = pb + (flip_b ? 2 * npb : 0u), *pb2 = pb + (flip_b ? 0u : 2 * npb);
  if (A_GLOBAL) {
    pa0 = uniform_ptr(pa0); pa1 = uniform_ptr(pa1); pa2 = uniform_ptr(pa2);
  }
  constexpr bool kByCount = !MASKED && !ONLY_LAST;
  const uint32_t lane_in_wave = ind0 & 63u;
  uint32_t n_full = 0, rem = 0;
  if (kByCount) {
    const uint32_t first = ind0 - lane_in_wave;
    const uint32_t have = n_ind > first ? n_ind - first : 0u;
    n_full = (uint32_t)__builtin_amdgcn_readfirstlane((int)(have >> 6 < (uint32_t)SLOTS ? have >> 6 : (uint32_t)SLOTS));
    rem = (uint32_t)__builtin_amdgcn_readfirstlane((int)(have >> 6 < (uint32_t)SLOTS ? have & 63u : 0u));
    vbits = ((1u << n_full) - 1u) | ((lane_in_wave < rem ? 1u : 0u) << n_full);
  }
#pragma unroll
  for (int j = 0; j < SLOTS; ++j) {
    const uint32_t ia = ia0 + (uint32_t)j * 64, ib = ib0 + (uint32_t)j * 64;
    typedef const __attribute__((address_space(1))) double gdouble_t;
    const bool in_regs = a_regs != nullptr && j < n_a_regs;
    const double a0 = in_regs ? a_regs[j < n_a_regs ? j : 0][0] : (A_GLOBAL ? ((gdouble_t *)pa0)[ia] : pa0[ia]),
                 a1 = in_regs ? a_regs[j < n_a_regs ? j : 0][1] : (A_GLOBAL ? ((gdouble_t *)pa1)[ia] : pa1[ia]),
                 a2 = in_regs ? a_regs[j < n_a_regs ? j : 0][2] : (A_GLOBAL ? ((gdouble_t *)pa2)[ia] : pa2[ia]);
    const double b0 = pb0[ib], b1 = pb[npb + ib], b2 = pb2[ib];
    const bool inb = kByCount ? ((vbits >> j) & 1u) != 0
                              : ((ONLY_LAST && j < SLOTS - 1) ? true : ind0 + (uint32_t)j * 64 < n_ind);
    if (!kByCount) {
      bool ok = inb;
      if (MASKED) ok = inb && !miss_data(a0, a1, a2) && !miss_data(b0, b1, b2);
      vbits |= (ok ? 1u : 0u) << j;
    }
    double z0 = a0, z1 = a1, z2 = a2;
    if (MASKED) {
      const double keep = ((vbits >> j) & 1u) ? 1.0 : 0.0;
      z0 = a0 * keep; z1 = a1 * keep; z2 = a2 * keep;
      P[j][0] = fma(z0, b0, 1.0 - keep);
    } else if (ONLY_LAST && j == SLOTS - 1) {
      P[j][0] = fma(a0, b0, inb ? 0.0 : 1.0);
    } else {
      P[j][0] = a0 * b0;
    }
    P[j][1] = z0 * b1; P[j][2] = z0 * b2;
    P[j][3] = z1 * b0; P[j][4] = z1 * b1; P[j][5] = z1 * b2;
    P[j][6] = z2 * b0; P[j][7] = z2 * b1; P[j][8] = z2 * b2;
    if (UNCENTRED && !MASKED) {
      sxy += fma(4.0, P[j][8], fma(2.0, P[j][5] + P[j][7], P[j][4]));
    } else if (UNCENTRED) {
      sxy = fma(fma(2.0, a2, a1), fma(2.0, b2, b1), sxy);
    } else {
      const double c1 = inb ? fma(2.0, a2, a1) - mean1 : 0.0;
      const double c2 = inb ? fma(2.0, b2, b1) - mean2 : 0.0;
      sxy = fma(c1, c2, sxy);
    }
  }
  if (kByCount) {
#pragma unroll
    for (int j = 0; j < SLOTS; ++j) {
      if (n_full <= (uint32_t)j) {
        const bool keep = n_full == (uint32_t)j && lane_in_wave < rem;
        P[j][0] = keep ? P[j][0] : 1.0;
      }
    }
  }
}

template <int SLOTS>
__device__ __forceinline__ uint32_t count_valid(uint32_t vbits) {
  uint32_t x = 0;
#pragma unroll
  for (int j = 0; j < SLOTS; ++j) x += (uint32_t)__popcll(__ballot((vbits >> j) & 1u));
  return x;
}

template <int SLOTS, int WAVES>
__device__ __forceinline__ uint32_t em_pair(const double (&P)[SLOTS][9], uint32_t vbits, double inv_x, double m1,
                                            double m2, double &f0, double &f1, double &f2, double &f3,
                                            double (*xch)[WAVES][4], int sub, int lane, int *status,
                                            uint32_t *xpar = nullptr) {
  static_assert(WAVES == 1 || WAVES == 2 || WAVES == 4 || WAVES == 8, "em_pair: 1, 2, 4 or 8 wavefronts per pair");
  f0 = (1 - m1) * (1 - m2); f1 = (1 - m1) * m2; f2 = m1 * (1 - m2); f3 = m1 * m2;
  if (m1 < 0 || m1 > 1 || m2 < 0 || m2 > 1) {
    if (lane == 0 && sub == 0) atomicExch(status, (int)NGSLD_ERR_MAF_RANGE);
    f0 = f1 = f2 = f3 = __builtin_nan("");
  }
  asm("" : "+v"(inv_x));
  bool bad = false, tie = false;
  uint32_t n_iter = 0;
  constexpr bool kTree = SLOTS > 1;
  constexpr bool kScaled = WAVES == 1;
  auto em_step = [&](auto tree_tag, auto drop_tag, double &n0, double &n1, double &n2, double &n3) {
    constexpr bool kShared = decltype(tree_tag)::value;
    constexpr bool kDrop = decltype(drop_tag)::value;
    static_assert(!kShared || (kTree && kDrop), "the shared-reciprocal step: several slots, three-value form");
    const double p00 = f0 * f0, p01 = f0 * f1, p02 = f0 * f2, p03 = f0 * f3, p11 = f1 * f1;
    const double p12 = f1 * f2, p13 = f1 * f3, p22 = f2 * f2, p23 = f2 * f3, p33 = f3 * f3;
    const double w1 = p01 + p01, w3 = p02 + p02, w4 = 2.0 * (p03 + p12), w5 = p13 + p13, w7 = p23 + p23;
    double R0 = 0, R1 = 0, R2 = 0, R3 = 0, R4 = 0, R5 = 0, R6 = 0, R7 = 0, R8 = 0;
    if (NGSLD_SETPRIO && kShared) __builtin_amdgcn_s_setprio(NGSLD_PRIO_S);
    auto slot_s = [&](int j) -> double {
      double s = p00 * P[j][0];
      s = fma(w1, P[j][1], s); s = fma(p11, P[j][2], s);
      s = fma(w3, P[j][3], s); s = fma(w4, P[j][4], s); s = fma(w5, P[j][5], s);
      s = fma(p22, P[j][6], s); s = fma(w7, P[j][7], s); s = fma(p33, P[j][8], s);
      return s;
    };
    auto slot_acc = [&](int j, double r) {
      if (!kDrop) R0 = fma(P[j][0], r, R0);
      R1 = fma(P[j][1], r, R1); R2 = fma(P[j][2], r, R2);
      R3 = fma(P[j][3], r, R3); R4 = fma(P[j][4], r, R4); R5 = fma(P[j][5], r, R5);
      R6 = fma(P[j][6], r, R6); R7 = fma(P[j][7], r, R7); R8 = fma(P[j][8], r, R8);
    };
    if constexpr (kShared) {
      double sv[SLOTS], rv[SLOTS];
#pragma unroll
      for (int j = 0; j < SLOTS; ++j) sv[j] = slot_s(j);
      if (NGSLD_SETPRIO) __builtin_amdgcn_s_setprio(NGSLD_PRIO_TREE);
      double inv = rcp_refined(RcpTree<SLOTS>::prod(sv));
      if (kScaled) inv *= inv_x;
      RcpTree<SLOTS>::down(sv, inv, rv);
      if (NGSLD_SETPRIO) __builtin_amdgcn_s_setprio(NGSLD_PRIO_R);
#pragma unroll
      for (int j = 0; j < SLOTS; ++j) slot_acc(j, rv[j]);
      if (NGSLD_SETPRIO) __builtin_amdgcn_s_setprio(NGSLD_PRIO_SERIAL);
    } else {
#pragma unroll
      for (int j = 0; j < SLOTS; ++j) {
        if ((vbits >> j) & 1u) slot_acc(j, rcp_refined(slot_s(j)));
      }
    }
    double t0 = kDrop ? 0.0 : fma(p03, R4, fma(p02, R3, fma(p01, R1, p00 * R0)));
    double t1 = fma(p13, R5, fma(p12, R4, fma(p11, R2, p01 * R1)));
    double t2 = fma(p23, R7, fma(p22, R6, fma(p12, R4, p02 * R3)));
    double t3 = fma(p33, R8, fma(p23, R7, fma(p13, R5, p03 * R4)));
    if (WAVES > 1 && kDrop) {
      const double w = wave_sum3_rows(t1, t2, t3);
      const int par = (int)((*xpar)++ & 1u);
      const int row = lane >> 4;
      const uint32_t base = lds_addr(&xch[par][0][0]);
      if ((lane & 15) == 0 && row != 1)
        lds_post(base + (uint32_t)((row == 0 ? 0 : row - 1) * WAVES + sub) * 8u, w);
      lds_barrier();
      if constexpr (WAVES == 8) {
        double v;
        asm volatile("ds_read_b64 %0, %1\n\ts_waitcnt lgkmcnt(0)" : "=&v"(v) : "v"(base + (uint32_t)(lane & 31) * 8u) : "memory");
        v += dpp_mov<0xB1>(v);
        v += dpp_mov<0x4E>(v);
        v += dpp_mov<0x141>(v);
        t1 = read_lane(v, 0); t2 = read_lane(v, 8); t3 = read_lane(v, 16);
      } else {
        constexpr int kHalf = WAVES > 1 ? WAVES / 2 : 1;
        dbl2 q[3 * kHalf];
        lds_gather<3 * kHalf>(base, q);
        t1 = q[0][0] + q[0][1]; t2 = q[kHalf][0] + q[kHalf][1]; t3 = q[2 * kHalf][0] + q[2 * kHalf][1];
#pragma unroll
        for (int v = 1; v < kHalf; ++v) {
          t1 += q[v][0]; t2 += q[kHalf + v][0]; t3 += q[2 * kHalf + v][0];
          t1 += q[v][1]; t2 += q[kHalf + v][1]; t3 += q[2 * kHalf + v][1];
        }
      }
    } else {
      if (kDrop)
        wave_sum3(t1, t2, t3);
      else
        wave_sum4(t0, t1, t2, t3);
      if (WAVES > 1) {
        const int par = (int)((*xpar)++ & 1u);
        if (lane == 0) {
          xch[par][sub][0] = t0; xch[par][sub][1] = t1; xch[par][sub][2] = t2; xch[par][sub][3] = t3;
        }
        lds_barrier();
        t0 = t1 = t2 = t3 = 0.0;
        for (int w = 0; w < WAVES; ++w) {
          t0 += xch[par][w][0]; t1 += xch[par][w][1]; t2 += xch[par][w][2]; t3 += xch[par][w][3];
        }
      }
    }
    const bool scaled = kShared && kScaled;
    n1 = scaled ? t1 : t1 * inv_x; n2 = scaled ? t2 : t2 * inv_x; n3 = scaled ? t3 : t3 * inv_x;
    n0 = kDrop ? 1.0 - ((n1 + n2) + n3) : t0 * inv_x;
  };
  constexpr double kFullBelow = 0x1p-10;
  bool full = __builtin_amdgcn_ballot_w64(f0 < kFullBelow) != 0;
  bool done = false;
  while (!done && n_iter < (uint32_t)kIterMax) {
    if constexpr (kTree) {
      if (!full) {
        for (; n_iter < (uint32_t)kIterMax; ++n_iter) {
          double n0, n1, n2, n3;
          em_step(PairedTag(), PairedTag(), n0, n1, n2, n3);
          if (__builtin_amdgcn_ballot_w64(!(n1 < 2.0))) break;
          bool conv = false;
          if (__builtin_amdgcn_ballot_w64(fabs(n1 - f1) < kEpsilonTie)) {
            const double eps = fmax(fmax(fabs(n0 - f0), fabs(n1 - f1)), fmax(fabs(n2 - f2), fabs(n3 - f3)));
            conv = __builtin_amdgcn_ballot_w64(eps < kEpsilon) != 0;
            tie |= __builtin_amdgcn_ballot_w64(fabs(eps - kEpsilon) < kTieMargin) != 0;
          }
          f0 = n0; f1 = n1; f2 = n2; f3 = n3;
          if (conv) {
            done = true;
            break;
          }
          if (__builtin_amdgcn_ballot_w64(n0 < kFullBelow)) {
            full = true;
            ++n_iter;
            break;
          }
        }
        if (done || n_iter >= (uint32_t)kIterMax) break;
        if (full) continue;
        if (WAVES > 1) lds_barrier();
      }
    }
    double n0, n1, n2, n3;
    if (WAVES == 1 || full)
      em_step(SingleTag(), SingleTag(), n0, n1, n2, n3);
    else
      em_step(SingleTag(), PairedTag(), n0, n1, n2, n3);
    if (__builtin_amdgcn_ballot_w64(!(n1 < 2.0))) {
      bad = true;
      break;
    }
    const double eps = fmax(fmax(fabs(n0 - f0), fabs(n1 - f1)), fmax(fabs(n2 - f2), fabs(n3 - f3)));
    f0 = n0; f1 = n1; f2 = n2; f3 = n3;
    tie |= __builtin_amdgcn_ballot_w64(fabs(eps - kEpsilon) < kTieMargin) != 0;
    if (__builtin_amdgcn_ballot_w64(eps < kEpsilon)) break;
    ++n_iter;
    if (!full && __builtin_amdgcn_ballot_w64(f0 < kFullBelow)) full = true;
  }
  if (bad) f0 = f1 = f2 = f3 = __builtin_nan("");
  return n_iter | (tie ? kTieBit : 0u);
}

__device__ __forceinline__ bool near_rounding(double v, double d) {
  const double t = fabs(v) * 1e6;
  return fabs((t - floor(t)) - 0.5) < d * 1e6;
}

__device__ __forceinline__ bool near_float_midpoint(double x, double d) {
  const float f = (float)x;
  const double lo = 0.5 * ((double)f + (double)nextafterf(f, -__builtin_inff()));
  const double hi = 0.5 * ((double)f + (double)nextafterf(f, __builtin_inff()));
  return fabs(x - lo) <= d || fabs(x - hi) <= d;
}

__device__ __forceinline__ bool chi2_unsettled(double f0, double f1, double f2, double f3, double dh) {
  const double sA = f0 + f1, sB = f0 + f2;
  if (near_float_midpoint(sA, 2 * dh + 0x1p-53 * fabs(sA)) || near_float_midpoint(sB, 2 * dh + 0x1p-53 * fabs(sB))) return true;
  const float freq_A = (float)sA, freq_B = (float)sB;
  const float exp_hap[4] = {freq_A * freq_B, freq_A * (1 - freq_B), (1 - freq_A) * freq_B, (1 - freq_A) * (1 - freq_B)};
  const double h[4] = {f0, f1, f2, f3};
  float chi2 = 0;
  double err = 0;
  for (int i = 0; i < 4; i++) {
    const double e = (double)exp_hap[i];
    const double d = h[i] - e;
    if (e == 0) {
      if (fabs(h[i]) <= dh) return true;
      return false;
    }
    const double t = d * d / e;
    const double s = (double)chi2 + t;
    const double dd = dh + 0x1p-52 * fabs(d);
    const double ds = err + 2 * ((2 * fabs(d) * dd + dd * dd) / e + 0x1p-51 * t) + 0x1p-52 * fabs(s);
    chi2 = (float)s;
    if (near_float_midpoint(s, ds)) {
      const double up = (double)nextafterf(chi2, __builtin_inff()) - (double)chi2;
// ... 76 lines not shown
```

ngsld_amd/csrc/ld_kernel_run.h:

```cpp
#pragma once

#include "ld_run_pipeline.h"

namespace ngsld {

template <int SLOTS, bool MASKED, bool SKIP = false>
__global__ __launch_bounds__(256, 2) void pair_ld_run_kernel(PairArgs A) {
  constexpr int kSiteBytes = SLOTS * 64 * 3 * 8;
  constexpr int kBuf = kSiteBytes + 32;
  constexpr uint32_t kNp = SLOTS * 64;
  constexpr uint32_t kRing = SLOTS <= 9 ? 32 : 8;
  constexpr int kRingOff = kSiteBytes + 4 * kBuf;
  constexpr int kListOff = kRingOff + 4 * (int)(kRing * sizeof(RunResult));
  __shared__ __attribute__((aligned(16))) char smem[kListOff + sizeof(RunList)];
  static_assert(sizeof(smem) <= 81920, "run kernel: two workgroups per CU need <= 80 KB of LDS each");

  const int lane = threadIdx.x & 63;
  const int wave = __builtin_amdgcn_readfirstlane((int)(threadIdx.x >> 6));
  const Run run = A.runs[blockIdx.x];
  const Item *g_items = A.items_all + run.first_item;
  const uint32_t s1 = g_items[0].s1;
  const double m1 = A.sc4[4 * (uint64_t)s1], mean1 = A.sc4[4 * (uint64_t)s1 + 1], rsx1 = A.sc4[4 * (uint64_t)s1 + 2];
  const bool skip1 = SKIP && A.sc4[4 * (uint64_t)s1 + 3] != 0.0;
  char *lds_a = smem;
  char *lds_b = smem + kSiteBytes + wave * kBuf;
  RunResult *ring = reinterpret_cast<RunResult *>(smem + kRingOff) + wave * kRing;
  RunList *L = reinterpret_cast<RunList *>(smem + kListOff);

  dma_site_to_lds<SLOTS>(A.planes + (uint64_t)s1 * A.site_stride, lds_a, lane, wave, 4);
  build_run_list(L, g_items, run.n_items);
  const uint32_t n_kept = (uint32_t)__builtin_amdgcn_readfirstlane((int)L->base[run.n_items]);
  const uint32_t s2_base = (uint32_t)__builtin_amdgcn_readfirstlane((int)L->items[0].s2_begin);
  const uint64_t rec_base = g_items[0].first_record - A.out_base;

  struct Cand {
    uint32_t s2;
    uint64_t rec;
    bool ok;
  };
  auto claim_next = [&]() -> Cand {
    uint32_t j = 0;
    if (lane == 0) j = atomicAdd(&L->claim, 1u);
    j = (uint32_t)__builtin_amdgcn_readfirstlane((int)j);
    if (j >= n_kept) return Cand{0u, 0ull, false};
    const uint32_t off = (uint32_t)__builtin_amdgcn_readfirstlane((int)L->cand[j]);
    return Cand{s2_base + off, rec_base + j, true};
  };
  auto dma_site = [&](uint32_t s2) {
    dma_site_to_lds<SLOTS>(A.planes + (uint64_t)s2 * A.site_stride, lds_b, lane, 0, 1);
    if (lane < 2)
      __builtin_amdgcn_global_load_lds((glb_void_t *)(reinterpret_cast<const char *>(A.sc4 + 4 * (uint64_t)s2) + lane * 16),
                                       (lds_void_t *)(lds_b + kSiteBytes), 16, 0, 0);
  };
  auto flush = [&](uint32_t n) {
    if ((uint32_t)lane < n) {
      const RunResult r = ring[lane];
      write_pair(A, r.rec, r.f[0], r.f[1], r.f[2], r.f[3], r.sxy, rsx1, r.rsx2, r.x, r.n_iter);
    }
  };

  Cand cur = claim_next();
  if (cur.ok) dma_site(cur.s2);
  uint32_t held = 0;
  while (cur.ok) {
    const Cand nxt = claim_next();
    asm volatile("s_waitcnt vmcnt(0)" ::: "memory");
    const double *sc = reinterpret_cast<const double *>(lds_b + kSiteBytes);
    const double m2 = uniform(sc[0]), mean2 = uniform(sc[1]), rsx2 = uniform(sc[2]);
    const bool skip = SKIP && (skip1 || uniform(sc[3]) != 0.0);
    double P[SLOTS][9];
    uint32_t vbits;
    double sxy;
    const Relabel rl = relabel(m1, m2, mean1, mean2);
    stage_pair<SLOTS, MASKED, !MASKED, true>(reinterpret_cast<const double *>(lds_a), kNp, (uint32_t)lane,
                                             reinterpret_cast<const double *>(lds_b), kNp, (uint32_t)lane, (uint32_t)lane,
                                             A.n_ind, rl.mean1, rl.mean2, P, vbits, sxy, rl.flip1, rl.flip2);
    asm volatile("s_waitcnt lgkmcnt(0)" ::: "memory");
    if (nxt.ok) dma_site(nxt.s2);
    const uint32_t x = MASKED ? count_valid<SLOTS>(vbits) : A.n_ind;
    const double inv_x = MASKED ? 1.0 / (double)x : A.inv_n;
    sxy = fma(-(double)A.n_ind * rl.mean1, rl.mean2, wave_sum1_bcast(sxy));
    double f0, f1, f2, f3;
    uint32_t n_iter = 0;
    if (skip) {
      f0 = f1 = f2 = f3 = __builtin_nan("");
    } else {
      n_iter = em_pair<SLOTS, 1>(P, vbits, inv_x, rl.m1, rl.m2, f0, f1, f2, f3, (double (*)[1][4]) nullptr, 0, lane, A.status);
      unrelabel(rl.flip1, rl.flip2, f0, f1, f2, f3);
    }
    if (lane == 0) {
      RunResult &r = ring[held];
      r.f[0] = f0; r.f[1] = f1; r.f[2] = f2; r.f[3] = f3;
      r.sxy = sxy;
      r.rsx2 = rsx2;
      r.x = x;
      r.n_iter = n_iter;
      r.rec = cur.rec;
    }
    if (++held == kRing) {
      flush(held);
      held = 0;
    }
    cur = nxt;
  }
  flush(held);
}

}
```

ngsld_amd/csrc/ld_pair_w1.hip:

```cpp
#include <cstdlib>

#include <algorithm>
#include <cstring>

#include "ld_kernel_run.h"
#include "ld_kernel_group.h"
#include "ld_kernel_stream.h"
#include "ld_dispatch.h"
#include "knobs.h"

namespace ngsld {

bool pair_config(uint64_t n_ind, PairConfig *cfg, int choice, bool masked) {
  if (n_ind == 0 || n_ind >= 0xffffffc0ull) return false;
  cfg->group = 64;
  cfg->waves = 1;
  cfg->form = 0;
  if (choice == kChooseABMulti || choice == kChooseAuto) {
    for (int w = 2; w <= 8; w *= 2) {
      const uint64_t slots = (n_ind + (uint64_t)w * 64 - 1) / ((uint64_t)w * 64);
      const uint64_t lo = choice == kChooseABMulti ? 9 : (!masked && w == 2 ? 11 : 9);
      const uint64_t hi = choice == kChooseABMulti ? 15 : (masked ? (w == 2 ? 13 : 14) : 15);
      if (slots >= lo && slots <= hi) {
        cfg->kernel = kMulti;
        cfg->form = 1;
        cfg->waves = w;
        cfg->slots = (int)slots;
        cfg->np = (uint32_t)(slots * (uint64_t)w * 64);
        return true;
      }
    }
  }
  if (n_ind > 5120u) {
    cfg->kernel = kStream;
    cfg->waves = choice == kChoosePlainStream ? 4 : 8;
    cfg->slots = 0;
    cfg->np = (uint32_t)((n_ind + 63) / 64 * 64);
    return true;
  }
  const bool g32 = n_ind > 128 && n_ind <= 256 && (((n_ind + 31) / 32) & 1ull);
  if (n_ind <= 128 || g32) {
    cfg->kernel = kGroup;
    cfg->group = n_ind <= 64 ? 8 : (n_ind <= 128 ? 16 : 32);
    cfg->slots = (int)((n_ind + (uint64_t)cfg->group - 1) / (uint64_t)cfg->group);
    cfg->np = (uint32_t)(cfg->slots * cfg->group);
    return true;
  }
  const uint64_t slots1 = (n_ind + 63) / 64;
  const bool want_ab = choice == kChooseAB && n_ind > 512 && n_ind <= 1024;
  if (!want_ab && (n_ind <= 512 || (choice == kChooseAuto && slots1 <= 10))) {
    cfg->kernel = kRun;
    cfg->slots = (int)slots1;
    cfg->np = (uint32_t)(slots1 * 64);
    return true;
  }
  if (want_ab || (choice == kChooseAuto && slots1 <= 15)) {
    cfg->kernel = kRunAB;
    cfg->slots = (int)slots1;
    cfg->np = (uint32_t)(slots1 * 64);
    return true;
  }
  int w = 2;
  while ((n_ind + 64ull * w - 1) / (64ull * w) > 8) w *= 2;
  const uint64_t half = (n_ind + 32ull * w - 1) / (32ull * w);
  if (w >= 4 && (half == 9 || half == 10)) w /= 2;
  cfg->waves = w;
  cfg->slots = (int)((n_ind + 64ull * w - 1) / (64ull * w));
  cfg->np = (uint32_t)(cfg->slots * w * 64);
  cfg->kernel = kMulti;
  return true;
}

template <int G, int SLOTS>
static hipError_t launch_g(bool masked, const PairArgs &a, hipStream_t stream) {
  if (a.n_runs == 0) return hipSuccess;
  if (a.n_runs > 0x7fffffffull) return hipErrorInvalidValue;
  const dim3 grid((unsigned)a.n_runs), block(256);
  if (masked)
    hipLaunchKernelGGL((pair_ld_group_kernel<G, SLOTS, true>), grid, block, 0, stream, a);
  else
    hipLaunchKernelGGL((pair_ld_group_kernel<G, SLOTS, false>), grid, block, 0, stream, a);
  return hipGetLastError();
}

template <int G>
static hipError_t launch_group(int slots, bool masked, const PairArgs &a, hipStream_t stream) {
  switch (slots) {
    case 1: return launch_g<G, 1>(masked, a, stream);
    case 2: return launch_g<G, 2>(masked, a, stream);
    case 3: return launch_g<G, 3>(masked, a, stream);
    case 4: return launch_g<G, 4>(masked, a, stream);
    case 5: return launch_g<G, 5>(masked, a, stream);
    case 6: return launch_g<G, 6>(masked, a, stream);
    case 7: return launch_g<G, 7>(masked, a, stream);
    case 8: return launch_g<G, 8>(masked, a, stream);
    default: return hipErrorInvalidValue;
  }
}

template <int SLOTS>
static hipError_t launch_run(bool masked, const PairArgs &a, hipStream_t stream) {
  if (a.n_runs == 0) return hipSuccess;
  if (a.n_runs > 0x7fffffffull) return hipErrorInvalidValue;
  const dim3 grid((unsigned)a.n_runs), block(256);
  if (a.skip_degenerate && a.flags != nullptr) {
    if (masked)
      hipLaunchKernelGGL((pair_ld_run_kernel<SLOTS, true, true>), grid, block, 0, stream, a);
    else
      hipLaunchKernelGGL((pair_ld_run_kernel<SLOTS, false, true>), grid, block, 0, stream, a);
    return hipGetLastError();
  }
  if (masked) {
    hipLaunchKernelGGL((pair_ld_run_kernel<SLOTS, true>), grid, block, 0, stream, a);
    return hipGetLastError();
  }
  hipLaunchKernelGGL((pair_ld_run_kernel<SLOTS, false>), grid, block, 0, stream, a);
  return hipGetLastError();
}

hipError_t launch_pair_wn(int slots, int waves, bool masked, const PairArgs &a, hipStream_t stream);

static hipError_t launch_pair_chunk(const PairConfig &cfg, bool masked, const PairArgs &a, hipStream_t stream);

hipError_t launch_pair_kernel(const PairConfig &cfg, bool masked, const PairArgs &a, hipStream_t stream) {
  uint64_t max_blocks = 1ull << 22;
  if (const char *e = test_knob("MAX_BLOCKS")) {
    const uint64_t u = std::strtoull(e, nullptr, 10);
    if (u >= 1 && u < max_blocks) max_blocks = u;
  }
  if (cfg.kernel == kMulti && cfg.waves > 1 && a.h_item_off != nullptr && a.item_off != nullptr && a.row1 > a.row0 &&
      !test_knob_is("TILES", "0")) {
    uint64_t longest = 0;
    for (uint32_t r = a.row0; r < a.row1; ++r) longest = std::max<uint64_t>(longest, a.h_item_off[r + 1] - a.h_item_off[r]);
    const uint64_t min_items = 32;
    uint64_t min_bytes = 256ull << 20;
    if (const char *e = test_knob("TILE_MIN_MB")) min_bytes = std::strtoull(e, nullptr, 10) << 20;
    if (longest >= min_items && a.planes_bytes >= min_bytes) {
      const uint32_t kTileRows = 64, kGroupRows = 512;
      for (uint32_t g0 = a.row0; g0 < a.row1; g0 += kGroupRows) {
        const uint32_t g1 = std::min<uint32_t>(a.row1, g0 + kGroupRows);
        uint64_t most = 0;
        for (uint32_t r = g0; r < g1; ++r) most = std::max<uint64_t>(most, a.h_item_off[r + 1] - a.h_item_off[r]);
        if (most == 0) continue;
        PairArgs b = a;
        b.row0 = g0;
        b.row1 = g1;
        b.tile_rows = kTileRows;
        b.tile_nk = (uint32_t)((most + 7) / 8);
        const uint64_t row_blocks = (g1 - g0 + kTileRows - 1) / kTileRows;
        const uint64_t blocks = row_blocks * b.tile_nk * kTileRows * 8ull;
        if (blocks > max_blocks) {
          b.tile_nk = 0;
          const uint64_t first = a.h_item_off[g0], count = a.h_item_off[g1] - first;
          for (uint64_t off = 0; off < count; off += max_blocks) {
            b.items = a.items_all + first + off;
            b.n_items = std::min<uint64_t>(max_blocks, count - off);
            const hipError_t e = launch_pair_chunk(cfg, masked, b, stream);
            if (e != hipSuccess) return e;
          }
          continue;
        }
        b.n_items = blocks;
        const hipError_t e = launch_pair_chunk(cfg, masked, b, stream);
        if (e != hipSuccess) return e;
      }
      return hipSuccess;
    }
  }
  const bool by_runs = uses_runs(cfg.kernel);
  const uint64_t total = by_runs ? a.n_runs : a.n_items;
  for (uint64_t off = 0; off < total; off += max_blocks) {
    PairArgs b = a;
    const uint64_t n = total - off < max_blocks ? total - off : max_blocks;
    if (by_runs) {
      b.runs = a.runs + off;
      b.n_runs = n;
    } else {
      b.items = a.items + off;
      b.n_items = n;
    }
    const hipError_t e = launch_pair_chunk(cfg, masked, b, stream);
    if (e != hipSuccess) return e;
  }
  return hipSuccess;
}

static hipError_t launch_pair_chunk(const PairConfig &cfg, bool masked, const PairArgs &a, hipStream_t stream) {
  if (cfg.kernel == kStream) {
    if (a.n_items == 0) return hipSuccess;
    if (a.n_items > 0x7fffffffull) return hipErrorInvalidValue;
    if (cfg.waves == 8) return launch_pair_bres((int)((a.np / 64u + 7u) / 8u), masked, a, stream);
    if (masked)
      hipLaunchKernelGGL((pair_ld_stream_kernel<true>), dim3((unsigned)a.n_items), dim3(256), 0, stream, a);
    else
      hipLaunchKernelGGL((pair_ld_stream_kernel<false>), dim3((unsigned)a.n_items), dim3(256), 0, stream, a);
    return hipGetLastError();
  }
// ... 30 lines not shown
```

ngsld_amd/csrc/ld_prep.h:

```cpp
#pragma once

#include "ld_common.h"

namespace ngsld {

struct PrepArgs {
  const double *raw;
  uint64_t site0;
  const double *maf_in;
  double *planes;
  uint64_t site_stride;
  uint64_t n_sites;
  uint32_t np, n_ind;
  int log_scale, ignore_miss, normalised_input;
  int text_semantics, call_geno;
  int exact_chain;
  double N_thresh, call_thresh;
  double *maf, *mean_e, *rsx;
  int *status;
  int *odd_missing;
  double missing_canon;
};

hipError_t launch_prep(const PrepArgs &a, hipStream_t stream);
struct ItemArgs {
  const uint32_t *row_end;
  const uint8_t *keep;
  const uint64_t *row_seed;
  const uint64_t *row_off;
  const uint64_t *item_off;
  uint64_t *row_count;
  Item *items;
  uint32_t n_sites, span;
  double rnd_sample;
  int count_only;
};
hipError_t launch_items(const ItemArgs &a, hipStream_t stream);
hipError_t launch_pack_scalars(const double *maf, const double *mean_e, const double *rsx, const uint8_t *skip, double *sc4, uint64_t n,
                               hipStream_t stream);
hipError_t launch_site_skip(const double *planes, uint64_t site_stride, uint32_t np, uint32_t n_ind, int ignore_miss, const double *maf,
                            uint64_t n_sites, uint8_t *skip, uint32_t *count, hipStream_t stream);
hipError_t launch_selftest(const double *in, double *out, hipStream_t stream);

}
```

ngsld_amd/csrc/ld_prep.hip:

```cpp
#include "ld_prep.h"
#include "taus.h"

namespace ngsld {

__device__ __forceinline__ double logsum3(double g0, double g1, double g2) {
  double M = g0;
  M = g1 >= M ? g1 : M;
  M = g2 >= M ? g2 : M;
  if (M == -__builtin_inf()) return -__builtin_inf();
  double sum = 0.0;
  sum += exp(g0 - M);
  sum += exp(g1 - M);
  sum += exp(g2 - M);
  return log(sum) + M;
}

__device__ __forceinline__ double conv_log(double g) {
  g = log(g);
  return g == -__builtin_inf() ? -1e15 : g;
}

__device__ __forceinline__ void call_geno(double &g0, double &g1, double &g2, double N_thresh, double call_thresh) {
  int max_pos = 0;
  double mx = -__builtin_inf();
// ... 105 lines not shown

__device__ __forceinline__ PrepFlags prep_flags(const PrepArgs &A) {
  PrepFlags F;
  F.log_scale = A.log_scale != 0;
  F.ignore_miss = A.ignore_miss != 0;
  F.text_semantics = A.text_semantics != 0;
  F.call_geno = A.call_geno != 0;
  F.fast_ok = !F.log_scale && !F.text_semantics && !F.call_geno && A.exact_chain == 0;
  F.N_thresh = A.N_thresh;
  F.call_thresh = A.call_thresh;
  return F;
}

__device__ __forceinline__ double site_rsx(double sq) { return 1.0 / sqrt(sq); }
__device__ __forceinline__ uint64_t triple_key(double g0, double g1, double g2) {
  const uint64_t a = (uint64_t)__double_as_longlong(g0), b = (uint64_t)__double_as_longlong(g1), c = (uint64_t)__double_as_longlong(g2);
  return a ^ ((b << 21) | (b >> 43)) ^ ((c << 42) | (c >> 22));
}
constexpr double kSumTol = 0x1p-40;
__device__ __forceinline__ bool odd_triple(double a0, double a1, double a2) { return !(fabs((a0 + a1 + a2) - 1.0) <= kSumTol); }
__device__ __forceinline__ double signed_rsx(double rsx, bool odd, double maf) { return (odd && maf > 0.5 - 1e-9) ? -rsx : rsx; }

template <int MAXJ>
__global__ __launch_bounds__(256) void prep_sites_wave_kernel(PrepArgs A) {
  const int lane = threadIdx.x & 63, wave = threadIdx.x >> 6;
  const PrepFlags F = prep_flags(A);
  for (uint64_t site = (uint64_t)blockIdx.x * 4 + wave; site < A.n_sites; site += (uint64_t)gridDim.x * 4) {
    const double *__restrict__ raw = A.raw + site * (uint64_t)A.n_ind * 3;
    double *__restrict__ pl = A.planes + (A.site0 + site) * A.site_stride;
    double e[MAXJ];
    double num = 0.0, den = 0.0, esum = 0.0;
    double mn = __builtin_inf(), mx = -__builtin_inf();
    uint64_t kmin = ~0ull, kmax = 0ull;
    bool nan_seen = false, odd = false;
#pragma unroll
    for (int j = 0; j < MAXJ; ++j) {
      const uint32_t i = (uint32_t)lane + 64u * (uint32_t)j;
      e[j] = 0.0;
      if (i < A.np) {
        double a0 = 0.0, a1 = 0.0, a2 = 0.0;
        if (i < A.n_ind) {
          const double g0 = raw[3 * (uint64_t)i], g1 = raw[3 * (uint64_t)i + 1], g2 = raw[3 * (uint64_t)i + 2];
          const uint64_t key = triple_key(g0, g1, g2);
          kmin = key < kmin ? key : kmin;
          kmax = key > kmax ? key : kmax;
          if (!A.normalised_input) {
            prep_individual(F, g0, g1, g2, a0, a1, a2, num, den, nan_seen);
          } else {
            a0 = g0;
            a1 = g1;
            a2 = g2;
          }
          odd = odd || odd_triple(a0, a1, a2);
          const double ev = fma(2.0, a2, a1);
          e[j] = ev;
          esum += ev;
          mn = ev < mn ? ev : mn;
          mx = ev > mx ? ev : mx;
        }
        pl[i] = a0;
        pl[A.np + i] = a1;
        pl[2 * (uint64_t)A.np + i] = a2;
      }
    }
    wave_sum3(num, den, esum);
    for (int off = 32; off > 0; off >>= 1) {
      const double x = __shfl_xor(mn, off), y = __shfl_xor(mx, off);
      mn = x < mn ? x : mn;
      mx = y > mx ? y : mx;
      const uint64_t p = (uint64_t)__shfl_xor((long long)kmin, off), q = (uint64_t)__shfl_xor((long long)kmax, off);
      kmin = p < kmin ? p : kmin;
      kmax = q > kmax ? q : kmax;
    }
    const double mean = mn == mx ? mn : esum / (double)A.n_ind;
    double sq = 0.0;
#pragma unroll
    for (int j = 0; j < MAXJ; ++j) {
      const uint32_t i = (uint32_t)lane + 64u * (uint32_t)j;
      const double d = i < A.n_ind ? e[j] - mean : 0.0;
      sq = fma(d, d, sq);
    }
    sq = wave_sum1(sq);
    const bool any_odd = __ballot(odd) != 0;
    if (lane == 0) {
      const double maf = A.normalised_input ? A.maf_in[site] : num / den;
      A.maf[A.site0 + site] = maf;
      A.mean_e[A.site0 + site] = mean;
      double rsx = signed_rsx(site_rsx(sq), any_odd, maf);
      if (mn == mx && kmin != kmax && !A.normalised_input) rsx = -__builtin_inf();
      A.rsx[A.site0 + site] = rsx;
    }
    if (nan_seen) atomicExch(A.status, (int)NGSLD_ERR_NAN);
  }
}

__global__ __launch_bounds__(256) void prep_sites_kernel(PrepArgs A) {
  __shared__ double sh3[4][3];
  __shared__ double sh1[4][1];
  const PrepFlags F = prep_flags(A);
  for (uint64_t site = blockIdx.x; site < A.n_sites; site += gridDim.x) {
    const double *__restrict__ raw = A.raw + site * (uint64_t)A.n_ind * 3;
    double *__restrict__ pl = A.planes + (A.site0 + site) * A.site_stride;
    double acc[3] = {0.0, 0.0, 0.0};
    double mn[1] = {__builtin_inf()}, mx[1] = {-__builtin_inf()};
    uint64_t key0 = 0;
    bool have_key = false, differs = false;
    bool nan_seen = false, odd = false;
    for (uint32_t i = threadIdx.x; i < A.np; i += 256) {
      double a0 = 0.0, a1 = 0.0, a2 = 0.0;
      if (i < A.n_ind) {
        const double g0 = raw[3 * (uint64_t)i], g1 = raw[3 * (uint64_t)i + 1], g2 = raw[3 * (uint64_t)i + 2];
        const uint64_t key = triple_key(g0, g1, g2);
        if (!have_key) {
          key0 = key;
          have_key = true;
        } else if (key != key0) {
          differs = true;
        }
        if (!A.normalised_input) {
          prep_individual(F, g0, g1, g2, a0, a1, a2, acc[0], acc[1], nan_seen);
        } else {
          a0 = g0;
          a1 = g1;
          a2 = g2;
        }
        odd = odd || odd_triple(a0, a1, a2);
        const double ev = fma(2.0, a2, a1);
        acc[2] += ev;
        mn[0] = ev < mn[0] ? ev : mn[0];
        mx[0] = ev > mx[0] ? ev : mx[0];
      }
      pl[i] = a0;
      pl[A.np + i] = a1;
      pl[2 * (uint64_t)A.np + i] = a2;
    }
    block_sum<3>(acc, sh3);
    block_minmax(mn, mx, sh1);
    const double mean = mn[0] == mx[0] ? mn[0] : acc[2] / (double)A.n_ind;
    double sq[1] = {0.0};
    for (uint32_t i = threadIdx.x; i < A.n_ind; i += 256) {
      const double d = fma(2.0, pl[2 * (uint64_t)A.np + i], pl[A.np + i]) - mean;
      sq[0] = fma(d, d, sq[0]);
    }
    block_sum<1>(sq, sh1);
    const bool any_odd = __syncthreads_or(odd ? 1 : 0) != 0;
    const uint64_t first_key = triple_key(raw[0], raw[1], raw[2]);
    const bool raw_differs = __syncthreads_or((differs || (have_key && key0 != first_key)) ? 1 : 0) != 0;
    if (threadIdx.x == 0) {
      const double maf = A.normalised_input ? A.maf_in[site] : acc[0] / acc[1];
      A.maf[A.site0 + site] = maf;
      A.mean_e[A.site0 + site] = mean;
      double rsx = signed_rsx(site_rsx(sq[0]), any_odd, maf);
      if (mn[0] == mx[0] && raw_differs && !A.normalised_input) rsx = -__builtin_inf();
      A.rsx[A.site0 + site] = rsx;
    }
    if (nan_seen) atomicExch(A.status, (int)NGSLD_ERR_NAN);
  }
}

__global__ __launch_bounds__(256) void missing_check_kernel(const double *__restrict__ raw, uint64_t n_triples, double canon, int *odd) {
  const uint64_t T = (uint64_t)gridDim.x * blockDim.x;
  const unsigned long long cb = (unsigned long long)__double_as_longlong(canon);
  bool bad = false;
  for (uint64_t t = (uint64_t)blockIdx.x * blockDim.x + threadIdx.x; t < n_triples; t += T) {
    const double g0 = raw[3 * t], g1 = raw[3 * t + 1], g2 = raw[3 * t + 2];
    const double mn = fmin(g0, fmin(g1, g2)), mx = fmax(g0, fmax(g1, g2));
// ... 202 lines not shown
```

Measured before the change: 206.8 million.

## Precompute first EM step for all pairs with an FP64 MFMA GEMM pre-pass

Adds a pre-pass that builds per-site planes (posterior u and expected genotype) during prep. A tiled FP64 MFMA kernel then computes, for every window pair, the cross-products that feed the first EM iteration and the covariance sum. The unmasked run kernel gets a FIRST variant that reads these precomputed values, skipping the first EM iteration and the wave reduction for sxy. The cost is extra memory for the planes and a per-chunk output buffer, an extra kernel launch per chunk, and a host sync when packing scalars.

```diff
diff --git a/include/ngsld.h b/include/ngsld.h
--- a/include/ngsld.h
+++ b/include/ngsld.h
@@ -125,6 +125,7 @@
 int ngsld_last_kernel_time(ngsld_ctx *ctx, double *total_ms, uint64_t *n_launches, uint64_t *n_pairs);
 
 const char *ngsld_pair_kernel(const ngsld_ctx *ctx);
+int ngsld_first_step(const ngsld_ctx *ctx);
 int ngsld_describe_dispatch(uint64_t n_ind, int ignore_miss_data, char *buf, size_t buf_len);
 
 int ngsld_set_tuning(ngsld_ctx *ctx, uint32_t pairs_per_item, uint64_t batch_pairs);
diff --git a/ngsld_amd/capi.py b/ngsld_amd/capi.py
--- a/ngsld_amd/capi.py
+++ b/ngsld_amd/capi.py
@@ -77,7 +77,7 @@
     "ngsld_set_replay_source", "ngsld_set_replay_matrix", "ngsld_set_replay", "ngsld_replay_stats", "ngsld_finish_device",
     "ngsld_set_exact_store", "ngsld_replay_info",
     "ngsld_plan_parts", "ngsld_run_multi", "ngsld_multi_last_distribution", "ngsld_rccl_selftest",
-    "ngsld_last_kernel_time", "ngsld_pair_kernel", "ngsld_describe_dispatch", "ngsld_set_tuning", "ngsld_selftest", "ngsld_selftest_format",
+    "ngsld_last_kernel_time", "ngsld_pair_kernel", "ngsld_first_step", "ngsld_describe_dispatch", "ngsld_set_tuning", "ngsld_selftest", "ngsld_selftest_format",
     "ngsld_selftest_printed", "ngsld_reserve_text_buffers",
     "ngsld_window_ends", "ngsld_plan_slabs", "ngsld_slab_sites_for_budget", "ngsld_sites_for_budget", "ngsld_streamed_replay_info", "ngsld_set_memory_budget", "ngsld_device_memory", "ngsld_run_streamed", "ngsld_run_streamed_text",
     "ngsld_host_read_geno_bin_range",
@@ -233,6 +233,9 @@
             L.ngsld_selftest_printed.argtypes = [vp, u64, vp, C.c_int32, C.c_int32, dbl, vp, vp, vp, vp]
         L.ngsld_window_ends.argtypes = [vp, u64, C.POINTER(Params), vp]
         L.ngsld_plan_slabs.argtypes = [vp, u64, C.POINTER(Params), u64, vp, u64, C.POINTER(u64)]
+        if hasattr(L, "ngsld_first_step"):
+            L.ngsld_first_step.argtypes = [C.c_void_p]
+            L.ngsld_first_step.restype = C.c_int
         L.ngsld_slab_sites_for_budget.argtypes = [u64, u64]
         L.ngsld_slab_sites_for_budget.restype = u64
         if hasattr(L, "ngsld_sites_for_budget"):
@@ -940,6 +943,9 @@
     def pair_kernel(self) -> str:
         return self._L.ngsld_pair_kernel(self._h).decode()
 
+    def first_step(self) -> bool:
+        return bool(self._L.ngsld_first_step(self._h))
+
     def last_kernel_time(self) -> tuple[float, int, int]:
         ms, nl, npairs = C.c_double(), C.c_uint64(), C.c_uint64()
         self._check(self._L.ngsld_last_kernel_time(self._h, C.byref(ms), C.byref(nl), C.byref(npairs)))
diff --git a/ngsld_amd/csrc/engine.h b/ngsld_amd/csrc/engine.h
--- a/ngsld_amd/csrc/engine.h
+++ b/ngsld_amd/csrc/engine.h
@@ -27,6 +27,7 @@
 #include "../../include/ngsld.h"
 #include "ld_common.h"
 #include "ld_dispatch.h"
+#include "ld_first_step.h"
 #include "ld_mean.h"
 #include "ld_prep.h"
 #include "ld_replay.h"
@@ -247,6 +248,11 @@
   uint32_t h_skip_count = 0;
   bool skip_on = true;
   bool skip_kernels = false;
+  bool first_on = true;
+  bool first_ok = false;
+  DevBuf<double> d_first_planes, d_sum_u, d_sc4f;
+  DevBuf<double> d_first[2];
+  uint64_t first_cap_items = 1ull << 22;
 
   bool planned = false;
   ngsld_params params{};
@@ -469,6 +475,9 @@
 int build_runs(ngsld_ctx *c, uint64_t run_len, const std::vector<uint64_t> &launch_ends);
 
 hipError_t timed_launch(ngsld_ctx *c, const PairArgs &a, hipStream_t stream);
+constexpr uint64_t kFirstBytesPerItem = 64ull * 2 * sizeof(double);
+constexpr uint64_t kFirstCapItems = 1ull << 22;
+int pack_first_scalars(ngsld_ctx *c);
 PairArgs make_args(ngsld_ctx *c, uint64_t r0, uint64_t r1, ngsld_rec_std *d_std, ngsld_rec_ext *d_ext,
                    uint32_t *d_flags = nullptr, uint32_t flag_cap = 0, uint64_t flag_n = 0);
 
diff --git a/ngsld_amd/csrc/engine.hip b/ngsld_amd/csrc/engine.hip
--- a/ngsld_amd/csrc/engine.hip
+++ b/ngsld_amd/csrc/engine.hip
@@ -69,6 +69,17 @@
   HIP_TRY(c, c->d_sc4.resize(4 * n_sites));
   HIP_TRY(c, c->d_status.resize(1));
   HIP_TRY(c, hipMemsetAsync(c->d_status.p, 0, sizeof(int), c->stream));
+  c->first_ok = false;
+  const bool want_first = c->first_on && cfg.kernel == kRun && cfg.slots >= 2 && !normalised && !ignore_miss;
+  if (want_first) {
+    HIP_TRY(c, c->d_first_planes.resize((size_t)n_sites * 2 * c->np));
+    HIP_TRY(c, c->d_sum_u.resize(n_sites));
+    HIP_TRY(c, c->d_sc4f.resize(4 * n_sites));
+  } else {
+    c->d_first_planes.release();
+    c->d_sum_u.release();
+    c->d_sc4f.release();
+  }
 
   PrepArgs a{};
   a.planes = c->d_planes.p;
@@ -90,6 +101,10 @@
   a.mean_e = c->d_mean.p;
   a.rsx = c->d_rsx.p;
   a.status = c->d_status.p;
+  if (want_first) {
+    a.first_planes = c->d_first_planes.p;
+    a.sum_u = c->d_sum_u.p;
+  }
   c->missing_canonical = false;
   const bool look_for_odd_missing = o.text_semantics && log_scale && !o.call_geno && !normalised;
   if (look_for_odd_missing) {
@@ -202,7 +217,22 @@
     c->d_hard_masks.release();
     c->d_hard_u.release();
   }
+  if (want_first && c->cfg.kernel == kRun) {
+    const int rcf = pack_first_scalars(c);
+    if (rcf != NGSLD_OK) return rcf;
+    c->first_ok = true;
+  } else {
+    c->d_first_planes.release();
+    c->d_sum_u.release();
+    c->d_sc4f.release();
+  }
   c->have_geno = true;
+  return NGSLD_OK;
+}
+
+int pack_first_scalars(ngsld_ctx *c) {
+  HIP_TRY(c, launch_pack_first_scalars(c->d_maf.p, c->d_mean.p, c->d_rsx.p, c->d_sum_u.p, c->d_skip.p, c->d_sc4f.p, c->n_sites, c->stream));
+  HIP_TRY(c, hipStreamSynchronize(c->stream));
   return NGSLD_OK;
 }
 }
@@ -257,7 +287,10 @@
   if (const char *k = std::getenv("NGSLD_REPLAY_THREADS")) c->replay_threads = std::atoi(k);
   if (const char *k = std::getenv("NGSLD_REPLAY_DEVICE")) c->replay_device = std::strcmp(k, "0") != 0;
   if (const char *k = std::getenv("NGSLD_REPLAY_SKIP")) c->skip_on = std::strcmp(k, "0") != 0;
+  if (const char *k = std::getenv("NGSLD_FIRST_STEP")) c->first_on = std::strcmp(k, "0") != 0;
   if (const char *k = std::getenv("NGSLD_EXACT_STORE")) c->exact_mode = std::max(0, std::min(2, std::atoi(k)));
+  if (const char *k = test_knob("FIRST_CAP_ITEMS"))
+    c->first_cap_items = std::min<uint64_t>(kFirstCapItems, std::max<uint64_t>(1, std::strtoull(k, nullptr, 10)));
   if (const char *k = test_knob("RUN_DIRECT")) c->run_direct = std::strcmp(k, "0") != 0;
   if (const char *k = test_knob("RUN_TAPER")) c->run_taper = std::strcmp(k, "0") != 0;
   if (const char *k = test_knob("RUN_STREAMS")) c->run_streams = std::atoi(k) >= 2 ? 2 : 1;
@@ -284,6 +317,7 @@
   if (c->exact_stream) (void)hipStreamDestroy(c->exact_stream);
   c->d_planes.release(); c->d_maf.release(); c->d_mean.release(); c->d_rsx.release(); c->d_sc4.release(); c->d_runs.release(); c->d_skip.release(); c->d_skip_count.release();
   c->d_hard_masks.release(); c->d_hard_u.release(); c->d_all_hard.release();
+  c->d_first_planes.release(); c->d_sum_u.release(); c->d_sc4f.release(); c->d_first[0].release(); c->d_first[1].release();
   c->d_xplanes.release(); c->d_xmaf.release(); c->d_xT.release(); c->d_xdepth.release(); c->d_xperm.release(); c->h_xstage[0].release(); c->h_xstage[1].release();
   c->lane_scratch_dev.release();
   for (int k = 0; k < ngsld_ctx::kSlots; ++k) c->lane_scratch[k].release();
@@ -367,6 +401,8 @@
     default: return "";
   }
 }
+
+int ngsld_first_step(const ngsld_ctx *c) { return (c != nullptr && c->have_geno && c->first_ok && c->first_on) ? 1 : 0; }
 
 int ngsld_describe_dispatch(uint64_t n_ind, int ignore_miss_data, char *buf, size_t buf_len) {
   if (buf == nullptr || buf_len == 0) return NGSLD_ERR_INVALID;
diff --git a/ngsld_amd/csrc/engine_plan.hip b/ngsld_amd/csrc/engine_plan.hip
--- a/ngsld_amd/csrc/engine_plan.hip
+++ b/ngsld_amd/csrc/engine_plan.hip
@@ -136,11 +136,19 @@
       if (site.maf != m && !(site.maf != site.maf && m != m)) {
         c->h_maf[s] = site.maf;
         changed = true;
+        if (c->first_ok && (site.maf > 0.5) != (m > 0.5)) {
+          const double nan = std::numeric_limits<double>::quiet_NaN();
+          HIP_TRY(c, hipMemcpy(c->d_sum_u.p + s, &nan, sizeof(double), hipMemcpyHostToDevice));
+        }
       }
     }
     if (changed) {
       HIP_TRY(c, hipMemcpy(c->d_maf.p, c->h_maf.data(), n * sizeof(double), hipMemcpyHostToDevice));
       HIP_TRY(c, launch_pack_scalars(c->d_maf.p, c->d_mean.p, c->d_rsx.p, c->d_skip.p, c->d_sc4.p, n, c->stream));
+      if (c->first_ok) {
+        const int rcf = pack_first_scalars(c);
+        if (rcf != NGSLD_OK) return rcf;
+      }
     }
   }
   plan_rows(c->h_pos_dist, c->h_maf, *p, n, c->h_row_end);
diff --git a/ngsld_amd/csrc/engine_run.hip b/ngsld_amd/csrc/engine_run.hip
--- a/ngsld_amd/csrc/engine_run.hip
+++ b/ngsld_amd/csrc/engine_run.hip
@@ -16,6 +16,45 @@
   auto &ev = c->ev_pool[c->ev_used++];
   hipError_t r = hipEventRecord(ev.first, stream);
   if (r != hipSuccess) return r;
+  if (c->first_ok && c->first_on && c->cfg.kernel == kRun && c->params.ignore_miss_data == 0 && a.n_runs > 0 && a.row1 > a.row0) {
+    DevBuf<double> &buf = c->d_first[stream == c->stream2 ? 1 : 0];
+    for (uint64_t r0 = a.row0; r0 < a.row1;) {
+      uint64_t r1 = r0 + 1;
+      while (r1 < a.row1 && c->h_item_off[r1 + 1] - c->h_item_off[r0] <= c->first_cap_items) ++r1;
+      const uint64_t item0 = c->h_item_off[r0], n_items = c->h_item_off[r1] - item0;
+      PairArgs b = a;
+      b.row0 = (uint32_t)r0;
+      b.row1 = (uint32_t)r1;
+      b.items = c->d_items.p + item0;
+      b.n_items = n_items;
+      b.runs = c->d_runs.p + c->h_run_off[r0];
+      b.n_runs = c->h_run_off[r1] - c->h_run_off[r0];
+      if (n_items > 0 && b.n_runs > 0) {
+        r = buf.resize(n_items * kFirstBytesPerItem / sizeof(double));
+        if (r != hipSuccess) return r;
+        FirstStepArgs f{};
+        f.ue = c->d_first_planes.p;
+        f.n_sites = c->n_sites;
+        f.np = c->np;
+        f.row0 = b.row0;
+        f.row1 = b.row1;
+        f.row_end = c->d_row_end.p;
+        f.item_off = c->d_item_off.p;
+        f.item0 = item0;
+        f.out = buf.p;
+        f.tiles = first_step_tiles(c->h_row_end.data(), r0, r1);
+        r = launch_first_step(f, stream);
+        if (r != hipSuccess) return r;
+        b.first = buf.p;
+        b.first_item0 = item0;
+        b.sc4 = c->d_sc4f.p;
+        r = launch_pair_kernel(c->cfg, false, b, stream);
+        if (r != hipSuccess) return r;
+      }
+      r0 = r1;
+    }
+    return hipEventRecord(ev.second, stream);
+  }
   r = launch_pair_kernel(c->cfg, c->params.ignore_miss_data != 0, a, stream);
   if (r != hipSuccess) return r;
   return hipEventRecord(ev.second, stream);
diff --git a/ngsld_amd/csrc/ld_common.h b/ngsld_amd/csrc/ld_common.h
--- a/ngsld_amd/csrc/ld_common.h
+++ b/ngsld_amd/csrc/ld_common.h
@@ -76,6 +76,8 @@
   const uint64_t *h_item_off;
   uint32_t row0, row1, tile_rows, tile_nk;
   uint64_t planes_bytes;
+  const double *first;
+  uint64_t first_item0;
 };
 
 typedef unsigned u32x2 __attribute__((ext_vector_type(2)));
diff --git a/ngsld_amd/csrc/ld_em.h b/ngsld_amd/csrc/ld_em.h
--- a/ngsld_amd/csrc/ld_em.h
+++ b/ngsld_amd/csrc/ld_em.h
@@ -139,11 +139,11 @@
   return x;
 }
 
-template <int SLOTS, int WAVES>
+template <int SLOTS, int WAVES, bool FIRST = false>
 __device__ __forceinline__ uint32_t em_pair(const double (&P)[SLOTS][9], uint32_t vbits, double inv_x, double m1,
                                             double m2, double &f0, double &f1, double &f2, double &f3,
                                             double (*xch)[WAVES][4], int sub, int lane, int *status,
-                                            uint32_t *xpar = nullptr) {
+                                            uint32_t *xpar = nullptr, double g = 0.0, double su1 = 0.0, double su2 = 0.0) {
   static_assert(WAVES == 1 || WAVES == 2 || WAVES == 4 || WAVES == 8, "em_pair: 1, 2, 4 or 8 wavefronts per pair");
   f0 = (1 - m1) * (1 - m2); f1 = (1 - m1) * m2; f2 = m1 * (1 - m2); f3 = m1 * m2;
   if (m1 < 0 || m1 > 1 || m2 < 0 || m2 > 1) {
@@ -249,6 +249,24 @@
   constexpr double kFullBelow = 0x1p-10;
   bool full = __builtin_amdgcn_ballot_w64(f0 < kFullBelow) != 0;
   bool done = false;
+  if constexpr (FIRST) {
+    static_assert(WAVES == 1 && kTree, "em_pair: the first step from the pre-pass is the run kernel's");
+    const double n3 = g * inv_x;
+    double n2 = su1 * inv_x - n3, n1 = su2 * inv_x - n3;
+    n2 = n2 < 0.0 ? 0.0 : n2;
+    n1 = n1 < 0.0 ? 0.0 : n1;
+    const double n0 = 1.0 - ((n1 + n2) + n3);
+    if (!__builtin_amdgcn_ballot_w64(!(n1 < 2.0) || !(n2 < 2.0) || !(n3 < 2.0) || f0 != f0)) {
+      const double eps = fmax(fmax(fabs(n0 - f0), fabs(n1 - f1)), fmax(fabs(n2 - f2), fabs(n3 - f3)));
+      done = __builtin_amdgcn_ballot_w64(eps < kEpsilon) != 0;
+      tie |= __builtin_amdgcn_ballot_w64(fabs(eps - kEpsilon) < kTieMargin) != 0;
+      f0 = n0; f1 = n1; f2 = n2; f3 = n3;
+      if (!done) {
+        n_iter = 1;
+        full = __builtin_amdgcn_ballot_w64(n0 < kFullBelow) != 0;
+      }
+    }
+  }
   while (!done && n_iter < (uint32_t)kIterMax) {
     if constexpr (kTree) {
       if (!full) {
diff --git a/ngsld_amd/csrc/ld_first_step.h b/ngsld_amd/csrc/ld_first_step.h
--- /dev/null
+++ b/ngsld_amd/csrc/ld_first_step.h
@@ -0,0 +1,24 @@
+#pragma once
+
+#include "ld_common.h"
+
+namespace ngsld {
+
+struct FirstStepArgs {
+  const double *ue;
+  uint64_t n_sites;
+  uint32_t np;
+  uint32_t row0, row1;
+  const uint32_t *row_end;
+  const uint64_t *item_off;
+  uint64_t item0;
+  double *out;
+  uint32_t tiles;
+};
+
+uint32_t first_step_tiles(const uint32_t *h_row_end, uint64_t row0, uint64_t row1);
+hipError_t launch_first_step(const FirstStepArgs &a, hipStream_t stream);
+hipError_t launch_pack_first_scalars(const double *maf, const double *mean_e, const double *rsx, const double *sum_u, const uint8_t *skip,
+                                     double *sc4f, uint64_t n, hipStream_t stream);
+
+}
diff --git a/ngsld_amd/csrc/ld_first_step.hip b/ngsld_amd/csrc/ld_first_step.hip
--- /dev/null
+++ b/ngsld_amd/csrc/ld_first_step.hip
@@ -0,0 +1,110 @@
+#include "ld_first_step.h"
+
+#include <algorithm>
+
+namespace ngsld {
+
+typedef double dbl4 __attribute__((ext_vector_type(4)));
+
+__global__ __launch_bounds__(256) void first_step_kernel(FirstStepArgs A) {
+  const int lane = threadIdx.x & 63;
+  const int wave = __builtin_amdgcn_readfirstlane((int)(threadIdx.x >> 6));
+  const uint32_t block = blockIdx.x / A.tiles, tile = blockIdx.x % A.tiles;
+  const uint32_t rb = A.row0 + block * 64u;
+  uint32_t end = 0;
+  if (rb + (uint32_t)lane < A.row1) end = A.row_end[rb + (uint32_t)lane];
+  for (int off = 32; off > 0; off >>= 1) {
+    const uint32_t o = (uint32_t)__shfl_xor((int)end, off);
+    end = o > end ? o : end;
+  }
+  end = (uint32_t)__builtin_amdgcn_readfirstlane((int)end);
+  const uint64_t c0 = (uint64_t)rb + 1u + 64ull * tile;
+  const uint64_t rw = (uint64_t)rb + 32u * (uint32_t)(wave >> 1), cw = c0 + 32u * (uint32_t)(wave & 1);
+  if (cw >= end || cw + 31u <= rw || rw >= A.row1) return;
+
+  const uint32_t i = (uint32_t)lane & 15u, g = (uint32_t)lane >> 4;
+  const uint64_t last = A.n_sites - 1, stride = 2ull * A.np;
+  const double *pa[2], *pb[2];
+#pragma unroll
+  for (int t = 0; t < 2; ++t) {
+    pa[t] = A.ue + std::min<uint64_t>(rw + 16u * t + i, last) * stride + 4u * g;
+    pb[t] = A.ue + std::min<uint64_t>(cw + 16u * t + i, last) * stride + 4u * g;
+  }
+  dbl4 accG[2][2], accE[2][2];
+#pragma unroll
+  for (int a = 0; a < 2; ++a)
+#pragma unroll
+    for (int b = 0; b < 2; ++b) accG[a][b] = accE[a][b] = dbl4{0.0, 0.0, 0.0, 0.0};
+  const uint32_t np = A.np;
+  for (uint32_t k0 = 0; k0 < np; k0 += 16) {
+    dbl4 au[2], ae[2], bu[2], be[2];
+#pragma unroll
+    for (int t = 0; t < 2; ++t) {
+      au[t] = *reinterpret_cast<const dbl4 *>(pa[t] + k0);
+      ae[t] = *reinterpret_cast<const dbl4 *>(pa[t] + np + k0);
+      bu[t] = *reinterpret_cast<const dbl4 *>(pb[t] + k0);
+      be[t] = *reinterpret_cast<const dbl4 *>(pb[t] + np + k0);
+    }
+#pragma unroll
+    for (int kk = 0; kk < 4; ++kk)
+#pragma unroll
+      for (int a = 0; a < 2; ++a)
+#pragma unroll
+        for (int b = 0; b < 2; ++b) {
+          accG[a][b] = __builtin_amdgcn_mfma_f64_16x16x4f64(au[a][kk], bu[b][kk], accG[a][b], 0, 0, 0);
+          accE[a][b] = __builtin_amdgcn_mfma_f64_16x16x4f64(ae[a][kk], be[b][kk], accE[a][b], 0, 0, 0);
+        }
+  }
+  typedef double dbl2 __attribute__((ext_vector_type(2)));
+#pragma unroll
+  for (int a = 0; a < 2; ++a)
+#pragma unroll
+    for (int r = 0; r < 4; ++r) {
+      const uint64_t row = rw + 16u * a + g + 4u * r;
+      if (row >= A.row1) continue;
+      const uint64_t row_end = A.row_end[row];
+      dbl2 *out = reinterpret_cast<dbl2 *>(A.out) + 64ull * (A.item_off[row] - A.item0);
+#pragma unroll
+      for (int b = 0; b < 2; ++b) {
+        const uint64_t col = cw + 16u * b + i;
+        if (col > row && col < row_end) out[col - row - 1] = dbl2{accG[a][b][r], accE[a][b][r]};
+      }
+    }
+}
+
+uint32_t first_step_tiles(const uint32_t *h_row_end, uint64_t row0, uint64_t row1) {
+  uint64_t widest = 0;
+  for (uint64_t rb = row0; rb < row1; rb += 64) {
+    uint64_t end = 0;
+    for (uint64_t r = rb; r < std::min<uint64_t>(rb + 64, row1); ++r) end = std::max<uint64_t>(end, h_row_end[r]);
+    if (end > rb + 1) widest = std::max<uint64_t>(widest, end - (rb + 1));
+  }
+  return (uint32_t)((widest + 63) / 64);
+}
+
+hipError_t launch_first_step(const FirstStepArgs &a, hipStream_t stream) {
+  if (a.row1 <= a.row0 || a.tiles == 0) return hipSuccess;
+  const uint64_t blocks = ((uint64_t)(a.row1 - a.row0) + 63) / 64 * a.tiles;
+  if (blocks > 0x7fffffffull) return hipErrorInvalidValue;
+  hipLaunchKernelGGL(first_step_kernel, dim3((unsigned)blocks), dim3(256), 0, stream, a);
+  return hipGetLastError();
+}
+
+__global__ void pack_first_scalars_kernel(const double *maf, const double *mean_e, const double *rsx, const double *sum_u,
+                                          const uint8_t *skip, double *sc4f, uint64_t n) {
+  const uint64_t s = (uint64_t)blockIdx.x * blockDim.x + threadIdx.x;
+  if (s >= n) return;
+  sc4f[4 * s] = maf[s];
+  sc4f[4 * s + 1] = mean_e[s];
+  sc4f[4 * s + 2] = rsx[s];
+  sc4f[4 * s + 3] = (skip != nullptr && skip[s]) ? -fabs(sum_u[s]) : fabs(sum_u[s]);
+}
+
+hipError_t launch_pack_first_scalars(const double *maf, const double *mean_e, const double *rsx, const double *sum_u, const uint8_t *skip,
+                                     double *sc4f, uint64_t n, hipStream_t stream) {
+  if (n == 0) return hipSuccess;
+  hipLaunchKernelGGL(pack_first_scalars_kernel, dim3((unsigned)((n + 255) / 256)), dim3(256), 0, stream, maf, mean_e, rsx, sum_u, skip, sc4f, n);
+  return hipGetLastError();
+}
+
+}
diff --git a/ngsld_amd/csrc/ld_kernel_run.h b/ngsld_amd/csrc/ld_kernel_run.h
--- a/ngsld_amd/csrc/ld_kernel_run.h
+++ b/ngsld_amd/csrc/ld_kernel_run.h
@@ -4,7 +4,7 @@
 
 namespace ngsld {
 
-template <int SLOTS, bool MASKED, bool SKIP = false>
+template <int SLOTS, bool MASKED, bool SKIP = false, bool FIRST = false>
 __global__ __launch_bounds__(256, 2) void pair_ld_run_kernel(PairArgs A) {
   constexpr int kSiteBytes = SLOTS * 64 * 3 * 8;
   constexpr int kBuf = kSiteBytes + 32;
@@ -21,7 +21,12 @@
   const Item *g_items = A.items_all + run.first_item;
   const uint32_t s1 = g_items[0].s1;
   const double m1 = A.sc4[4 * (uint64_t)s1], mean1 = A.sc4[4 * (uint64_t)s1 + 1], rsx1 = A.sc4[4 * (uint64_t)s1 + 2];
-  const bool skip1 = SKIP && A.sc4[4 * (uint64_t)s1 + 3] != 0.0;
+  static_assert(!FIRST || !MASKED, "run kernel: the first step from the pre-pass counts every individual");
+  const double sc1 = A.sc4[4 * (uint64_t)s1 + 3];
+  const bool skip1 = SKIP && (FIRST ? __double2hiint(sc1) < 0 : sc1 != 0.0);
+  const double su1 = FIRST ? fabs(sc1) : 0.0;
+  typedef const __attribute__((address_space(4))) dbl2 first_t;
+  const uint64_t first_base = FIRST ? 64ull * (run.first_item - A.first_item0) : 0ull;
   char *lds_a = smem;
   char *lds_b = smem + kSiteBytes + wave * kBuf;
   RunResult *ring = reinterpret_cast<RunResult *>(smem + kRingOff) + wave * kRing;
@@ -37,14 +42,19 @@
     uint32_t s2;
     uint64_t rec;
     bool ok;
+    uint32_t off;
   };
   auto claim_next = [&]() -> Cand {
     uint32_t j = 0;
     if (lane == 0) j = atomicAdd(&L->claim, 1u);
     j = (uint32_t)__builtin_amdgcn_readfirstlane((int)j);
-    if (j >= n_kept) return Cand{0u, 0ull, false};
+    if (j >= n_kept) return Cand{0u, 0ull, false, 0u};
     const uint32_t off = (uint32_t)__builtin_amdgcn_readfirstlane((int)L->cand[j]);
-    return Cand{s2_base + off, rec_base + j, true};
+    return Cand{s2_base + off, rec_base + j, true, off};
+  };
+  auto load_first = [&](const Cand &c) -> dbl2 {
+    if (!FIRST || !c.ok) return dbl2{0.0, 0.0};
+    return *reinterpret_cast<first_t *>((uintptr_t)(reinterpret_cast<const dbl2 *>(A.first) + (first_base + c.off)));
   };
   auto dma_site = [&](uint32_t s2) {
     dma_site_to_lds<SLOTS>(A.planes + (uint64_t)s2 * A.site_stride, lds_b, lane, 0, 1);
@@ -61,13 +71,16 @@
 
   Cand cur = claim_next();
   if (cur.ok) dma_site(cur.s2);
+  dbl2 ge = load_first(cur);
   uint32_t held = 0;
   while (cur.ok) {
     const Cand nxt = claim_next();
     asm volatile("s_waitcnt vmcnt(0)" ::: "memory");
     const double *sc = reinterpret_cast<const double *>(lds_b + kSiteBytes);
     const double m2 = uniform(sc[0]), mean2 = uniform(sc[1]), rsx2 = uniform(sc[2]);
-    const bool skip = SKIP && (skip1 || uniform(sc[3]) != 0.0);
+    const double sc2 = (SKIP || FIRST) ? uniform(sc[3]) : 0.0;
+    const bool skip = SKIP && (skip1 || (FIRST ? __double2hiint(sc2) < 0 : sc2 != 0.0));
+    const double su2 = FIRST ? fabs(sc2) : 0.0;
     double P[SLOTS][9];
     uint32_t vbits;
     double sxy;
@@ -77,15 +90,17 @@
                                              A.n_ind, rl.mean1, rl.mean2, P, vbits, sxy, rl.flip1, rl.flip2);
     asm volatile("s_waitcnt lgkmcnt(0)" ::: "memory");
     if (nxt.ok) dma_site(nxt.s2);
+    const dbl2 ge_nxt = load_first(nxt);
     const uint32_t x = MASKED ? count_valid<SLOTS>(vbits) : A.n_ind;
     const double inv_x = MASKED ? 1.0 / (double)x : A.inv_n;
-    sxy = fma(-(double)A.n_ind * rl.mean1, rl.mean2, wave_sum1_bcast(sxy));
+    sxy = fma(-(double)A.n_ind * rl.mean1, rl.mean2, FIRST ? ge[1] : wave_sum1_bcast(sxy));
     double f0, f1, f2, f3;
     uint32_t n_iter = 0;
     if (skip) {
       f0 = f1 = f2 = f3 = __builtin_nan("");
     } else {
-      n_iter = em_pair<SLOTS, 1>(P, vbits, inv_x, rl.m1, rl.m2, f0, f1, f2, f3, (double (*)[1][4]) nullptr, 0, lane, A.status);
+      n_iter = em_pair<SLOTS, 1, FIRST>(P, vbits, inv_x, rl.m1, rl.m2, f0, f1, f2, f3, (double (*)[1][4]) nullptr, 0, lane, A.status,
+                                        nullptr, ge[0], su1, su2);
       unrelabel(rl.flip1, rl.flip2, f0, f1, f2, f3);
     }
     if (lane == 0) {
@@ -102,6 +117,7 @@
       held = 0;
     }
     cur = nxt;
+    ge = ge_nxt;
   }
   flush(held);
 }
diff --git a/ngsld_amd/csrc/ld_pair_w1.hip b/ngsld_amd/csrc/ld_pair_w1.hip
--- a/ngsld_amd/csrc/ld_pair_w1.hip
+++ b/ngsld_amd/csrc/ld_pair_w1.hip
@@ -104,6 +104,12 @@
   if (a.n_runs > 0x7fffffffull) return hipErrorInvalidValue;
   const dim3 grid((unsigned)a.n_runs), block(256);
   if (a.skip_degenerate && a.flags != nullptr) {
+    if constexpr (SLOTS >= 2) {
+      if (a.first != nullptr && !masked) {
+        hipLaunchKernelGGL((pair_ld_run_kernel<SLOTS, false, true, true>), grid, block, 0, stream, a);
+        return hipGetLastError();
+      }
+    }
     if (masked)
       hipLaunchKernelGGL((pair_ld_run_kernel<SLOTS, true, true>), grid, block, 0, stream, a);
     else
@@ -113,6 +119,12 @@
   if (masked) {
     hipLaunchKernelGGL((pair_ld_run_kernel<SLOTS, true>), grid, block, 0, stream, a);
     return hipGetLastError();
+  }
+  if constexpr (SLOTS >= 2) {
+    if (a.first != nullptr) {
+      hipLaunchKernelGGL((pair_ld_run_kernel<SLOTS, false, false, true>), grid, block, 0, stream, a);
+      return hipGetLastError();
+    }
   }
   hipLaunchKernelGGL((pair_ld_run_kernel<SLOTS, false>), grid, block, 0, stream, a);
   return hipGetLastError();
diff --git a/ngsld_amd/csrc/ld_prep.h b/ngsld_amd/csrc/ld_prep.h
--- a/ngsld_amd/csrc/ld_prep.h
+++ b/ngsld_amd/csrc/ld_prep.h
@@ -20,6 +20,8 @@
   int *status;
   int *odd_missing;
   double missing_canon;
+  double *first_planes;
+  double *sum_u;
 };
 
 hipError_t launch_prep(const PrepArgs &a, hipStream_t stream);
diff --git a/ngsld_amd/csrc/ld_prep.hip b/ngsld_amd/csrc/ld_prep.hip
--- a/ngsld_amd/csrc/ld_prep.hip
+++ b/ngsld_amd/csrc/ld_prep.hip
@@ -211,6 +211,32 @@
     }
     sq = wave_sum1(sq);
     const bool any_odd = __ballot(odd) != 0;
+    if (A.first_planes != nullptr) {
+      const double maf = num / den;
+      const bool flip = maf > 0.5;
+      const double m = flip ? 1.0 - maf : maf, p0 = 1.0 - m;
+      const double w0 = p0 * p0, w1 = 2.0 * (p0 * m), w2 = m * m;
+      double *__restrict__ fp = A.first_planes + (A.site0 + site) * 2ull * A.np;
+      double usum = 0.0;
+#pragma unroll
+      for (int j = 0; j < MAXJ; ++j) {
+        const uint32_t i = (uint32_t)lane + 64u * (uint32_t)j;
+        if (i < A.np) {
+          double u = 0.0, ev = 0.0;
+          if (i < A.n_ind) {
+            const double z0 = pl[(flip ? 2ull * A.np : 0ull) + i], z1 = pl[A.np + i], z2 = pl[(flip ? 0ull : 2ull * A.np) + i];
+            const double sa = fma(w2, z2, fma(w1, z1, w0 * z0));
+            u = m * fma(m, z2, p0 * z1) / sa;
+            ev = fma(2.0, z2, z1);
+          }
+          fp[i] = u;
+          fp[A.np + i] = ev;
+          usum += u;
+        }
+      }
+      usum = wave_sum1(usum);
+      if (lane == 0) A.sum_u[A.site0 + site] = any_odd ? __builtin_nan("") : usum;
+    }
     if (lane == 0) {
       const double maf = A.normalised_input ? A.maf_in[site] : num / den;
       A.maf[A.site0 + site] = maf;
```

Result: faster. 223.0 million (median of 6 runs) (+7.8%).
